# CobaltCrabby/ray_tracer

Hardware: AMD Instinct MI355X
Metric: Mrays/s (reference-semantics closest-hit queries) at 1920x1080 Sponza (higher is better)
Workload: dtype f32; 1 GPU; sponza (synthetic-262267-tris), 1920x1080, 8 spp/step, bounceLimit 8, rows interleaved over 1 GPU(s), up to 10 steps in flight per rank (groups of 10+9+9+9); scene=sponza, assets=synthetic-262267-tris, width=1920, height=1080, frames_in_flight=10, pipeline=multi-kernel (k_trace_pw + k_shade per round)

## Files before the change

ray_tracer_amd/csrc/rt_device.hip:

```cpp

#include "rt_kernels.hip.h"
#include "bvh_build.hip.h"

#include <dlfcn.h>
#include <rccl/rccl.h>

#include <algorithm>
#include <chrono>
#include <cmath>
#include <cstdio>
#include <cstdlib>
#include <string>
#include <type_traits>
#include <vector>

namespace {

struct DevBuf {
    void* p = nullptr;
    size_t bytes = 0;
    DevBuf() = default;
    DevBuf(DevBuf&& o) noexcept : p(o.p), bytes(o.bytes) { o.p = nullptr; o.bytes = 0; }
    ~DevBuf() { release(); }
    void release() { if (p) (void)hipFree(p); p = nullptr; bytes = 0; }
};

struct EventPair { hipEvent_t a, b; };
#define RT_MAX_LANES 4
#define RT_FRAMES_MAX_SLOTS (24ull << 20)
struct RowsOf {
    uint32_t width = 0, height = 0, row0 = 0, rowStride = 0, nRows = 0;
    bool whole(uint32_t w, uint32_t h) const { return width == w && height == h && row0 == 0 && rowStride == 1 && nRows == h; }
};

}

struct rt_ctx {
    std::string error;
    int device = 0, numCUs = 256;
    hipStream_t ownStream = nullptr, stream = nullptr;
    DevScene sc{};
    std::vector<DevBuf> sceneBufs;
    DevBuf texelBuf, texInfoBuf, triUVBuf, objTreeBuf, objCostBuf;
    DevBuf matBuf, sphereBuf, sphereMatBuf, objInvBuf, objFwdBuf, objMetaBuf, objBoxBuf, objSkipBuf, maskBoxBuf, emitBuf, emitPreBuf;
    SceneSources host;
    DevBuf objAlphaBuf;
    uint32_t maxLeafDepth = 0;
    std::vector<RootInfo> rootOf;
    bool cull = false;
    ncclComm_t comm = nullptr;
    int commRanks = 0, commRank = 0;
    DevBuf gatherBuf;
    DevBuf stateBuf, queueBuf, fbBuf, counterBuf, scratchBuf;
    DevBuf overflowBuf[RT_MAX_LANES];
    hipStream_t sideStream[RT_MAX_LANES - 1] = {};
    hipEvent_t forkEvent = nullptr, joinEvent[RT_MAX_LANES - 1] = {}, pollEventSide[RT_MAX_LANES - 1] = {};
    uint32_t capacity = 0;
    PathState ps{}; Queues q{};
    uint32_t* hostCounts = nullptr;
    uint32_t fbPixels = 0; bool fbValid = false;
    bool profiling = false;
    std::vector<EventPair> evPool;
    size_t evUsed = 0;
    hipEvent_t profBase = nullptr;
    DevCounters* snap = nullptr;
    hipEvent_t snapEvent = nullptr;
    hipEvent_t pollEvent = nullptr;
    DevBuf probeBuf;
    DevBuf waveTimeBuf;
    DevBuf aovBuf, aovCounterBuf;
    DevBuf shadeStatBuf;
    uint32_t aovPixels = 0; bool aovValid = false;
    RowsOf fbRows, aovRows;
    DevBuf dnWorkBuf, dnHostBuf, dnOutBuf;
    size_t dnOutPixels = 0; bool dnValid = false;

    struct Tuning {
        int objTreeMin = 48;
        int framesPerLaunch = 0;
        uint64_t framesMaxSlots = RT_FRAMES_MAX_SLOTS;
        int cameraReuse = 1;
        int lightQueries = 1;
        int lanes = 3;
        bool lanesSet = false;
        uint32_t lanesMinSlots = 1u << 20;
        int laneGridPct = 0;
        int traceVariant = 1;
        int pipeline = -1;
        uint32_t fusedBelowPixels = 4000000;
        uint32_t fusedBelowBoxTests = 70;
        int refill = 8;
        int refillMk = 16;
        bool refillMkSet = false;
        int chunk = 256;
        int ldsStackCap = 24;
        int fastLanes = 32;
        bool fastLanesSet = false;
        int wSetup = 16, wLeaf = 16;
        bool wSetupSet = false, wLeafSet = false;
        int wSetupFused = 16, wLeafFused = 24;
        int blocksPerCU = 0;
        int phaseStats = 0;
        int tileSlots = 1;
        int fastShare = 10;
        int maskIdentity = 0;
        int scatter = -1;
        int hotPairs = 2;
        int pixelRefill = 0;
        int batchPixels = 0;
        int batchFixed = 80;
        int fusedMaps = 0;
        int probe = 1;
    } tune;

    struct Measured {
        bool snapPending = false;
        unsigned long long snapBox = 0, snapRays = 0, snapSeg = 0, snapPaths = 0;
        double boxPerRay = -1.0;
        double segPerPath = -1.0;
    } meas;

    struct Reports {
        int lastPipeline = 0;
        int lastParts = 1;
        char lastKernel[96] = "";
        size_t waveTimesCount = 0;
        double traceMs = 0.0;
        uint64_t traceLaunches = 0;
        std::vector<std::pair<float, float>> traceSpans;
        uint64_t traceLaunchesTotal = 0, aovLaunches = 0;
        double bvhBuildMs = 0.0;
    } rep;
    int fail(const std::string& m) { error = m; return -1; }
    int hip(hipError_t e, const char* what) {
        if (e == hipSuccess) return 0;
        error = std::string(what) + ": " + hipGetErrorString(e);
        return -(int)e - 1000;
    }
};

#define RT_HIP(ctx, call)                                    \
    do {                                                     \
        int _rc = (ctx)->hip((call), #call);                 \
        if (_rc) return _rc;                                 \
    } while (0)

namespace {

int dev_alloc(rt_ctx* c, DevBuf& b, size_t bytes) {
    if (b.p && b.bytes >= bytes) return 0;
    b.release();
    if (bytes == 0) bytes = 256;
    RT_HIP(c, hipMalloc(&b.p, bytes));
    b.bytes = bytes;
    return 0;
}

int upload(rt_ctx* c, DevBuf& b, const void* src, size_t bytes) {
    int rc = dev_alloc(c, b, bytes);
    if (rc) return rc;
    if (bytes) RT_HIP(c, hipMemcpyAsync(b.p, src, bytes, hipMemcpyHostToDevice, c->stream));
    RT_HIP(c, hipStreamSynchronize(c->stream));
    return 0;
}

template <typename T>
int upload_table(rt_ctx* c, DevBuf& b, const std::vector<T>& v, const T*& field) {
    int rc = upload(c, b, v.data(), v.size() * sizeof(T));
    if (rc) return rc;
    field = (const T*)b.p;
    return 0;
}

int ensure_state(rt_ctx* c, uint32_t nPixels) {
    if (c->capacity >= nPixels && c->stateBuf.p) return 0;
    const size_t stride4 = (((size_t)nPixels * 16) + 255) & ~(size_t)255;
    const size_t stride1 = (((size_t)nPixels * 4) + 255) & ~(size_t)255;
    const int nF4 = RT_STATE_F4_ARRAYS, nU1 = 2;
    int rc = dev_alloc(c, c->stateBuf, stride4 * nF4 + stride1 * nU1);
    if (rc) return rc;
    PathState& ps = c->ps;
    ps.base = (float4*)c->stateBuf.p;
    ps.pitch = (uint32_t)(stride4 / 16);
    ps.pitchStat = (uint32_t)(stride1 / 4);

    const size_t qa = (((size_t)nPixels * 4) + 255) & ~(size_t)255;
    const size_t qr = (((size_t)nPixels * 3 * 4) + 255) & ~(size_t)255;
    rc = dev_alloc(c, c->queueBuf, 2 * qa + 2 * qr + 256);
    if (rc) return rc;
    char* qb = (char*)c->queueBuf.p;
    c->q.active[0] = (uint32_t*)qb;
    c->q.active[1] = (uint32_t*)(qb + qa);
    c->q.rays[0] = (uint32_t*)(qb + 2 * qa);
    c->q.rays[1] = (uint32_t*)(qb + 2 * qa + qr);
    c->q.counts = (uint32_t*)(qb + 2 * qa + 2 * qr);
// ... 73 lines not shown
    return trace_pw_kernel<STACK, OVF, false, false, CULL>();
}

template <typename K>
uint32_t resident_blocks(const rt_ctx* c, K kernel) {
    int perCU = c->tune.blocksPerCU;
    if (perCU <= 0 && (hipOccupancyMaxActiveBlocksPerMultiprocessor(&perCU, kernel, RT_BLOCK, 0) != hipSuccess || perCU <= 0)) perCU = 4;
    return (uint32_t)perCU * (uint32_t)c->numCUs;
}

int overflow_buf(rt_ctx* c, const Dispatch& d, int stack, bool ovf, uint32_t resident, uint32_t** out) {
    *out = nullptr;
    if (!ovf || c->maxLeafDepth <= (uint32_t)stack) return 0;
    DevBuf& ob = c->overflowBuf[d.part];
    int rc = dev_alloc(c, ob, (size_t)(c->maxLeafDepth - stack) * resident * RT_BLOCK * 4);
    if (rc) return rc;
    *out = (uint32_t*)ob.p;
    return 0;
}

int wave_time_buf(rt_ctx* c, uint32_t blocks, unsigned long long** out) {
    c->rep.waveTimesCount = (size_t)blocks * (RT_BLOCK / RT_WAVE);
    int rc = dev_alloc(c, c->waveTimeBuf, c->rep.waveTimesCount * 16);
    if (rc) return rc;
    *out = (unsigned long long*)c->waveTimeBuf.p;
    return 0;
}

int prof_begin(rt_ctx* c, const Dispatch& d, EventPair** ev) {
    *ev = nullptr;
    if (!d.profiled) return 0;
    if (c->evUsed == c->evPool.size()) {
        EventPair p;
        RT_HIP(c, hipEventCreate(&p.a));
        RT_HIP(c, hipEventCreate(&p.b));
        c->evPool.push_back(p);
    }
    *ev = &c->evPool[c->evUsed++];
    RT_HIP(c, hipEventRecord((*ev)->a, d.stream));
    return 0;
}
int prof_end(rt_ctx* c, const Dispatch& d, EventPair* ev) {
    if (ev) RT_HIP(c, hipEventRecord(ev->b, d.stream));
    if (d.launches) ++*d.launches;
    return 0;
}

uint32_t fused_batch_pixels(const rt_ctx* c, uint32_t nPixels, uint32_t waves, uint32_t evenBelow) {
    if (c->tune.batchPixels > 0) return (uint32_t)std::min(c->tune.batchPixels, (int)RT_WAVE);
    if (((uint64_t)nPixels + RT_WAVE - 1) / RT_WAVE > (uint64_t)evenBelow * waves) return RT_WAVE;
    uint32_t best = RT_WAVE;
    uint64_t bestCost = ~0ull;
    for (uint32_t b = RT_WAVE; b >= 16; b--) {
        const uint64_t nb = (nPixels + b - 1) / b;
        const uint64_t rounds = (nb + waves - 1) / waves;
        const uint64_t cost = rounds * (uint64_t)((uint32_t)c->tune.batchFixed + b);
        if (cost < bestCost) { bestCost = cost; best = b; }
    }
    return best;
}

int launch_fused(rt_ctx* c, const Dispatch& d, const FrameParams& fp, float4* fb) {
    EventPair* ev;
    int rc = prof_begin(c, d, &ev);
    if (rc) return rc;
    const FusedChoice k = d.sc.mapFlags
        ? kernel_choice(d.pixStats ? k_render_fused_maps<true> : k_render_fused_maps<false>, k_render_fused_maps<false>, 24, true, "k_render_fused_maps<%s>", tf(d.pixStats))
        : with_stack<false>(c->maxLeafDepth, (uint32_t)c->tune.ldsStackCap, c->cull, [&](auto S, auto O, auto C) { return d.pixStats ? fused_kernel<S, O, true, C>() : fused_kernel<S, O, false, C>(); });
    const uint32_t resident = resident_blocks(c, k.occupancy);
    const uint32_t nSlots = (uint32_t)dispatch_slots(fp.nPixels, fp.nFrames);
    const uint64_t fewBelow = (c->meas.segPerPath >= 0.0 && c->meas.segPerPath < 2.5) ? 8ull : 5ull;
    const bool fewBlocks = ((uint64_t)nSlots + RT_WAVE - 1) / RT_WAVE < fewBelow * resident * (RT_BLOCK / RT_WAVE);
    const uint32_t pixelRefill = c->tune.pixelRefill > 0 ? (uint32_t)c->tune.pixelRefill
                               : ((c->meas.boxPerRay >= (double)c->tune.fusedBelowBoxTests || fewBlocks) ? 8u : (uint32_t)RT_WAVE);
    const uint32_t evenBelow = pixelRefill < RT_WAVE ? 1u : 2u;
    uint32_t batchPixels = fused_batch_pixels(c, nSlots, resident * (RT_BLOCK / RT_WAVE), evenBelow);
    const uint32_t wavesResident = resident * (RT_BLOCK / RT_WAVE);
    const uint32_t g = fp.nFrames > 1u ? 0u : c->tune.scatter >= 0 ? (uint32_t)c->tune.scatter : ((((uint64_t)nSlots + RT_WAVE - 1) / RT_WAVE <= (uint64_t)evenBelow * wavesResident) ? 4u : 0u);
    if (g) batchPixels = std::min((uint32_t)RT_WAVE, (batchPixels + g - 1) / g * g);
    const uint32_t nBatches = g ? ((nSlots + g - 1) / g + batchPixels / g - 1) / (batchPixels / g) : (nSlots + batchPixels - 1) / batchPixels;
    const uint32_t blocks = std::max(1u, std::min((nBatches + (RT_BLOCK / RT_WAVE) - 1) / (RT_BLOCK / RT_WAVE), resident));
    uint32_t* overflow;
    if ((rc = overflow_buf(c, d, k.stack, k.ovf, resident, &overflow))) return rc;
    RT_HIP(c, hipMemsetAsync(d.counts + 5, 0, 4, d.stream));
    const uint32_t fastLanes = c->tune.fastLanesSet ? (uint32_t)c->tune.fastLanes : (c->meas.boxPerRay >= (double)c->tune.fusedBelowBoxTests ? 40u : 24u);
    const uint32_t wLeaf = (uint32_t)c->tune.wLeafFused;
    unsigned long long* waveTimes = nullptr;
    if (d.phaseStats && (rc = wave_time_buf(c, blocks, &waveTimes))) return rc;
    FusedArgs fa{d.counts + 5, fb, (DevCounters*)c->counterBuf.p, overflow, (uint32_t)c->tune.refill, (uint32_t)c->tune.wSetupFused, wLeaf, fastLanes, batchPixels, g, (uint32_t)c->tune.fastShare, waveTimes, pixelRefill};
    const FusedKernArgs ka{d.sc, c->ps, fp, fa};
    memcpy(c->rep.lastKernel, k.name, sizeof k.name);
    hipLaunchKernelGGL(k.kernel, dim3(blocks), dim3(RT_BLOCK), 0, d.stream, ka);
    RT_HIP(c, hipGetLastError());
    return prof_end(c, d, ev);
}

template <int STACK>
void launch_v0_t(rt_ctx* c, const Dispatch& d, uint32_t maxRays, const TraceArgs& ta) {
    uint32_t blocks = (maxRays + RT_BLOCK - 1) / RT_BLOCK;
    snprintf(c->rep.lastKernel, sizeof c->rep.lastKernel, "k_trace<%d>", STACK);
    hipLaunchKernelGGL((k_trace<STACK>), dim3(blocks), dim3(RT_BLOCK), 0, d.stream, d.sc, c->ps, ta);
}

int launch_trace(rt_ctx* c, const Dispatch& d, uint32_t maxRays, const TraceArgs& ta) {
    if (maxRays == 0) return 0;
    EventPair* ev;
    int rc = prof_begin(c, d, &ev);
    if (rc) return rc;
    const uint32_t depth = c->maxLeafDepth;
    const bool pix = d.pixStats || ta.perRayBox;
    const bool alpha = d.sc.mapFlags & RT_MAP_ALPHA;
    if (!alpha && c->tune.traceVariant == 0) {
        if (depth <= 8) launch_v0_t<8>(c, d, maxRays, ta);
        else if (depth <= 16) launch_v0_t<16>(c, d, maxRays, ta);
        else if (depth <= 24) launch_v0_t<24>(c, d, maxRays, ta);
        else if (depth <= 32) launch_v0_t<32>(c, d, maxRays, ta);
        else if (depth <= 48) launch_v0_t<48>(c, d, maxRays, ta);
        else launch_v0_t<64>(c, d, maxRays, ta);
    } else {
        const bool tableWanted = c->tune.hotPairs && d.sc.hotNodes > 0 && !d.phaseStats && !pix;
        const uint32_t cap = (depth > 24u && c->tune.ldsStackCap >= 24 && tableWanted) ? 16u : (uint32_t)c->tune.ldsStackCap;
        const TracePwChoice k = alpha
            ? kernel_choice(pix ? k_trace_pw_alpha<true> : k_trace_pw_alpha<false>, k_trace_pw_alpha<false>, 24, true, "k_trace_pw_alpha<%s>", tf(pix))
            : with_stack<true>(depth, cap, c->cull, [&](auto S, auto O, auto C) { return choose_trace_pw<S, O, C>(c, d, pix); });
        const uint32_t resident = resident_blocks(c, k.occupancy);
        const uint32_t blocks = std::min((maxRays + RT_BLOCK - 1) / RT_BLOCK, std::max(1u, (uint32_t)((uint64_t)resident * (uint32_t)d.gridPct / 100u)));
        uint32_t* overflow;
        if ((rc = overflow_buf(c, d, k.stack, k.ovf, resident, &overflow))) return rc;
        unsigned long long* waveTimes = nullptr;
        const bool times = d.phaseStats == 1 || (d.phaseStats >= 2 && d.launches && *d.launches == (uint64_t)(d.phaseStats - 2));
        if (!alpha && times && (rc = wave_time_buf(c, blocks, &waveTimes))) return rc;
        const bool longRays = c->meas.boxPerRay >= (double)c->tune.fusedBelowBoxTests;
        const uint32_t refillMk = c->tune.refillMkSet ? (uint32_t)c->tune.refillMk : (longRays ? 12u : 16u);
        const uint32_t wSetup = c->tune.wSetupSet ? (uint32_t)c->tune.wSetup : (longRays ? 32u : 16u);
        const TracePwArgs pa{ta.queue, ta.count, d.counts + 4, refillMk, (uint32_t)c->tune.chunk, wSetup, (uint32_t)c->tune.wLeaf, (uint32_t)c->tune.fastLanes, (uint32_t)c->tune.fastShare,
                             ta.perRayBox, ta.perRayTri, ta.counters, (unsigned long long*)((char*)c->counterBuf.p + sizeof(DevCounters)), waveTimes, overflow, ta.countAux, ta.countAux2, ta.auxOffset};
        memcpy(c->rep.lastKernel, k.name, sizeof k.name);
        hipLaunchKernelGGL(k.kernel, dim3(blocks), dim3(RT_BLOCK), 0, d.stream, d.sc, c->ps, pa);
    }
    RT_HIP(c, hipGetLastError());
    return prof_end(c, d, ev);
}

void poll_ray_cost(rt_ctx* c) {
    if (!c->meas.snapPending || hipEventQuery(c->snapEvent) != hipSuccess) return;
    c->meas.snapPending = false;
    const unsigned long long box = c->snap->boxTests - c->snap->skippedBoxTests, rays = c->snap->raysTraced;
    if (rays > c->meas.snapRays && box >= c->meas.snapBox && rays - c->meas.snapRays > 100000ull)
        c->meas.boxPerRay = (double)(box - c->meas.snapBox) / (double)(rays - c->meas.snapRays);
    const unsigned long long seg = c->snap->segments, paths = c->snap->paths;
    if (paths > c->meas.snapPaths && seg >= c->meas.snapSeg && paths - c->meas.snapPaths > 100000ull) c->meas.segPerPath = (double)(seg - c->meas.snapSeg) / (double)(paths - c->meas.snapPaths);
    c->meas.snapBox = box;
    c->meas.snapRays = rays;
    c->meas.snapSeg = seg;
    c->meas.snapPaths = paths;
}
void request_ray_cost(rt_ctx* c) {
    if (c->meas.snapPending) return;
    if (hipMemcpyAsync(c->snap, c->counterBuf.p, sizeof(DevCounters), hipMemcpyDeviceToHost, c->stream) != hipSuccess) return;
    if (hipEventRecord(c->snapEvent, c->stream) != hipSuccess) return;
    c->meas.snapPending = true;
}
void measured_new_scene(rt_ctx* c) {
    if (c->meas.snapPending) { c->meas.snapBox = c->snap->boxTests; c->meas.snapRays = c->snap->raysTraced; c->meas.snapPending = false; }
    c->meas.boxPerRay = -1.0;
}

int harvest_events(rt_ctx* c) {
    for (size_t i = 0; i < c->evUsed; i++) {
        float ms = 0.f;
        RT_HIP(c, hipEventElapsedTime(&ms, c->evPool[i].a, c->evPool[i].b));
        c->rep.traceMs += ms;
        c->rep.traceLaunches++;
        float t0 = 0.f;
        if (c->profBase && hipEventElapsedTime(&t0, c->profBase, c->evPool[i].a) == hipSuccess) c->rep.traceSpans.emplace_back(t0, t0 + ms);
    }
    c->evUsed = 0;
    return 0;
}

int rebuild_emitters(rt_ctx* c) {
    c->sc.emitCount = 0; c->sc.emitSphereMask = 0; c->sc.emitMode = 0;
    const MapLayout maps = layout_maps(c->host, c->sc.texCount);
    int rc = upload_table(c, c->objAlphaBuf, maps.objAlpha, c->sc.objAlpha);
    if (rc) return rc;
    c->sc.mapFlags = maps.mapFlags;
    if (!c->tune.lightQueries) return 0;
    const EmitterLayout e = layout_emitters(c->host, c->rootOf, c->sc.texCount);
    if (!e.mode) return 0;
    if (!e.tris.empty()) {
        if ((rc = upload_table(c, c->emitBuf, e.tris, c->sc.emitTris))) return rc;
    } else {
        if ((rc = dev_alloc(c, c->emitBuf, 256))) return rc;
        c->sc.emitTris = (const uint2*)c->emitBuf.p;
    }
    if ((rc = dev_alloc(c, c->emitPreBuf, std::max<size_t>(e.tris.size(), 1) * 4 * sizeof(float4)))) return rc;
    if (!e.tris.empty()) {
        hipLaunchKernelGGL(k_emit_precompute, dim3(((uint32_t)e.tris.size() + 63u) / 64u), dim3(64), 0, c->stream, c->sc.triPos, c->sc.emitTris, (uint32_t)e.tris.size(), (float4*)c->emitPreBuf.p);
        RT_HIP(c, hipGetLastError());
        RT_HIP(c, hipStreamSynchronize(c->stream));
    }
    c->sc.emitPre = (const float4*)c->emitPreBuf.p;
    c->sc.emitCount = (uint32_t)e.tris.size();
    c->sc.emitSphereMask = e.sphereMask;
    c->sc.emitMode = 1;
    return 0;
}

int set_materials(rt_ctx* c, const RayMaterial* m, uint32_t n) {
    int rc = upload_table(c, c->matBuf, layout_materials(m, n), c->sc.mats);
    if (rc) return rc;
    c->sc.materialCount = n;
    c->host.mats.assign(m, m + n);
    return rebuild_emitters(c);
}

int set_spheres(rt_ctx* c, const Sphere* s, uint32_t n) {
    const SphereLayout l = layout_spheres(s, n);
    int rc = upload_table(c, c->sphereBuf, l.spheres, c->sc.spheres);
    if (rc) return rc;
    if ((rc = upload_table(c, c->sphereMatBuf, l.mat, c->sc.sphereMat))) return rc;
    c->sc.sphereCount = n;
    c->sc.sphereTestMask = l.testMask;
    c->host.sphereMat.assign(l.mat.begin(), l.mat.begin() + n);
    return rebuild_emitters(c);
}

int set_objects(rt_ctx* c, const ObjectLayout& l, const RenderObject* o, uint32_t n) {
    if (l.treeLevels && getenv("RT_DEBUG_OBJTREE")) dump_object_tree(l, n);
    int rc;
    if ((rc = upload_table(c, c->objInvBuf, l.inv, c->sc.objInv))) return rc;
    if ((rc = upload_table(c, c->objFwdBuf, l.fwd, c->sc.objFwd))) return rc;
    if ((rc = upload_table(c, c->objMetaBuf, l.meta, c->sc.objMeta))) return rc;
    if ((rc = upload_table(c, c->objBoxBuf, l.box, c->sc.objBox))) return rc;
    if ((rc = upload_table(c, c->maskBoxBuf, l.maskBox, c->sc.maskBox))) return rc;
    if ((rc = upload_table(c, c->objSkipBuf, l.skipCost, c->sc.objSkipCost))) return rc;
    if ((rc = upload_table(c, c->objTreeBuf, l.tree, c->sc.objTree))) return rc;
    if ((rc = upload_table(c, c->objCostBuf, l.cost, c->sc.objCost))) return rc;
    for (int k = 0; k <= RT_OBJTREE_LEVELS; k++) c->sc.objTreeOff[k] = l.treeOff[k];
    c->sc.objTreeLevels = l.treeLevels;
    c->sc.reachCount = l.reachCount;
    c->sc.maskBase = l.maskBase;
    c->sc.cullOriginLimit = l.cullOriginLimit;
    c->cull = l.cull;
    c->sc.objectCount = n;
    c->host.objMat.resize(n); c->host.objRoot.resize(n); c->host.objSampler.resize(n);
    for (uint32_t i = 0; i < n; i++) { c->host.objMat[i] = o[i].materialIndex; c->host.objRoot[i] = o[i].bvhIndex; c->host.objSampler[i] = o[i].samplerIndex; }
    return rebuild_emitters(c);
}

}

extern "C" {

int rt_device_count(int* out) {
    int n = 0;
    hipError_t e = hipGetDeviceCount(&n);
    if (out) *out = (e == hipSuccess) ? n : 0;
    return e == hipSuccess ? 0 : -1;
}

int rt_create(int device, rt_ctx** out) {
    if (!out) return -1;
    *out = nullptr;
    int n = 0;
    if (hipGetDeviceCount(&n) != hipSuccess || n <= 0) return -2;
    if (device < 0 || device >= n) return -3;
    if (hipSetDevice(device) != hipSuccess) return -4;
    rt_ctx* c = new rt_ctx();
    c->device = device;
    if (hipStreamCreateWithFlags(&c->ownStream, hipStreamNonBlocking) != hipSuccess) { c->ownStream = nullptr; rt_destroy(c); return -5; }
    c->stream = c->ownStream;
    {
        hipDeviceProp_t prop;
        if (hipGetDeviceProperties(&prop, device) == hipSuccess && prop.multiProcessorCount > 0) c->numCUs = prop.multiProcessorCount;
    }
    if (hipHostMalloc((void**)&c->hostCounts, 64, hipHostMallocDefault) != hipSuccess) { c->hostCounts = nullptr; rt_destroy(c); return -6; }
    if (hipHostMalloc((void**)&c->snap, sizeof(DevCounters), hipHostMallocDefault) != hipSuccess) { c->snap = nullptr; rt_destroy(c); return -6; }
    if (hipEventCreateWithFlags(&c->snapEvent, hipEventDisableTiming) != hipSuccess) { c->snapEvent = nullptr; rt_destroy(c); return -6; }
    if (hipEventCreateWithFlags(&c->pollEvent, hipEventDisableTiming) != hipSuccess) { c->pollEvent = nullptr; rt_destroy(c); return -6; }
    if (dev_alloc(c, c->counterBuf, sizeof(DevCounters) + 256) != 0) { rt_destroy(c); return -7; }
    (void)hipMemsetAsync(c->counterBuf.p, 0, sizeof(DevCounters) + 256, c->stream);
    if (dev_alloc(c, c->aovCounterBuf, sizeof(DevCounters)) != 0) { rt_destroy(c); return -7; }
    (void)hipMemsetAsync(c->aovCounterBuf.p, 0, sizeof(DevCounters), c->stream);
    if (dev_alloc(c, c->shadeStatBuf, sizeof(ShadeStatStripe) * RT_STAT_STRIPES) != 0) { rt_destroy(c); return -7; }
    (void)hipMemsetAsync(c->shadeStatBuf.p, 0, sizeof(ShadeStatStripe) * RT_STAT_STRIPES, c->stream);
    (void)hipStreamSynchronize(c->stream);
    *out = c;
    return 0;
}

void rt_destroy(rt_ctx* c) {
    if (!c) return;
    (void)hipSetDevice(c->device);
    if (c->stream) (void)hipStreamSynchronize(c->stream);
    (void)rt_comm_destroy(c);
    for (auto& e : c->evPool) { (void)hipEventDestroy(e.a); (void)hipEventDestroy(e.b); }
    if (c->hostCounts) (void)hipHostFree(c->hostCounts);
    if (c->snap) (void)hipHostFree(c->snap);
    for (hipEvent_t e : {c->snapEvent, c->pollEvent, c->forkEvent, c->profBase})
        if (e) (void)hipEventDestroy(e);
    for (int l = 0; l < RT_MAX_LANES - 1; l++) {
        if (c->joinEvent[l]) (void)hipEventDestroy(c->joinEvent[l]);
        if (c->pollEventSide[l]) (void)hipEventDestroy(c->pollEventSide[l]);
        if (c->sideStream[l]) (void)hipStreamDestroy(c->sideStream[l]);
    }
    if (c->ownStream) (void)hipStreamDestroy(c->ownStream);
    delete c;
}

const char* rt_last_error(const rt_ctx* c) { return c ? c->error.c_str() : "null ctx"; }

int rt_set_stream(rt_ctx* c, void* s) {
    if (!c) return -1;
    RT_HIP(c, hipStreamSynchronize(c->stream));
    c->stream = s ? (hipStream_t)s : c->ownStream;
    return 0;
}

int rt_upload_textures(rt_ctx* c, const RtTexture* tex, uint32_t n) {
    if (!c || (!tex && n)) return -1;
    const TextureLayout l = layout_textures(tex, n);
    if (!l.error.empty()) return c->fail(l.error);
    RT_HIP(c, hipSetDevice(c->device));
    int rc = upload_table(c, c->texelBuf, l.texels, c->sc.texels);
    if (rc) return rc;
    if ((rc = upload_table(c, c->texInfoBuf, l.info, c->sc.texInfo))) return rc;
    c->sc.texCount = n;
    return rebuild_emitters(c);
}

int rt_update_materials(rt_ctx* c, const RayMaterial* m, uint32_t n) {
    if (!c || (!m && n)) return -1;
    RT_HIP(c, hipSetDevice(c->device));
    return set_materials(c, m, n);
}

int rt_update_spheres(rt_ctx* c, const Sphere* s, uint32_t n) {
    if (!c || (!s && n)) return -1;
    RT_HIP(c, hipSetDevice(c->device));
    return set_spheres(c, s, n);
}

int rt_update_objects(rt_ctx* c, const RenderObject* o, uint32_t n) {
    if (!c || (!o && n)) return -1;
    if (c->rootOf.empty() && n) return c->fail("rt_update_objects before rt_upload_scene");
    const ObjectLayout l = layout_objects(o, n, c->rootOf, c->sc.materialCount, c->tune.objTreeMin, c->tune.maskIdentity);
    if (!l.error.empty()) return c->fail(l.error);
    RT_HIP(c, hipSetDevice(c->device));
    return set_objects(c, l, o, n);
}

int rt_upload_scene(rt_ctx* c, const RtSceneArrays* s) {
    if (!c || !s) return -1;
    SceneLayout l = layout_scene(*s, c->tune.objTreeMin, c->tune.maskIdentity);
    if (!l.error.empty()) return c->fail(l.error);
    MeshLayout& m = l.meshes;

    RT_HIP(c, hipSetDevice(c->device));
    RT_HIP(c, hipStreamSynchronize(c->stream));
    measured_new_scene(c);
    c->host = SceneSources{};
    c->sc.emitMode = 0; c->sc.emitCount = 0; c->sc.emitSphereMask = 0;
    c->sc.mapFlags = 0;
    c->sc.texCount = 0;
    c->sceneBufs.clear();
    c->sceneBufs.resize(5);
    int rc;
    if ((rc = upload_table(c, c->triUVBuf, m.triUV, c->sc.triUV))) return rc;
// ... 8 lines not shown
    c->maxLeafDepth = m.maxLeafDepth;
    c->rootOf = std::move(m.rootOf);

    if ((rc = set_materials(c, s->materials, s->materialCount))) return rc;
    if ((rc = set_spheres(c, s->spheres, s->sphereCount))) return rc;
    return set_objects(c, l.objects, s->objects, s->objectCount);
}

int rt_sync(rt_ctx* c) {
    if (!c) return -1;
    RT_HIP(c, hipStreamSynchronize(c->stream));
    return harvest_events(c);
}

}

namespace {
int check_tile(rt_ctx* c, const PushConstants* pc, uint32_t width, uint32_t height, uint32_t row0, uint32_t rowStride, uint32_t nRows,
               const char* fn) {
    if (width == 0 || height == 0 || rowStride == 0) return c->fail(std::string(fn) + ": bad image geometry");
    if (nRows && (uint64_t)row0 + (uint64_t)(nRows - 1) * rowStride >= height) return c->fail(std::string(fn) + ": rows exceed the image");
    if (!c->sc.nodes) return c->fail(std::string(fn) + " before rt_upload_scene");
    const RayTracerData& td = pc->rayTraceParams;
    if (td.sphereCount > c->sc.sphereCount) return c->fail("rayTraceParams.sphereCount exceeds the uploaded spheres");
    if (td.objectCount > c->sc.objectCount) return c->fail("rayTraceParams.objectCount exceeds the uploaded objects");
    return 0;
}

DevScene dispatch_scene(const rt_ctx* c, const RayTracerData& td) {
    DevScene sc = c->sc;
    sc.sphereCount = td.sphereCount;
    sc.objectCount = td.objectCount;
    if (sc.objectCount < c->sc.objectCount) { sc.reachCount = 0; sc.objTreeLevels = 0; }
    return sc;
}

FrameParams frame_camera(const rt_ctx* c, const PushConstants* pc, uint32_t width, uint32_t height, uint32_t row0, uint32_t rowStride,
                         uint32_t nRows, uint32_t nPixels) {
    FrameParams fp{};
    memcpy(fp.camRot, pc->camInfo.cameraRotation, 64);
    memcpy(fp.camPos, pc->camInfo.pos, 12);
    fp.planeHeight = pc->camInfo.nearPlane * rt_tan(rt_radians(pc->camInfo.fov * 0.5f)) * 2.f;
    fp.planeWidth = fp.planeHeight * pc->camInfo.aspectRatio;
    fp.bottomLeft[0] = -fp.planeWidth / 2.f;
    fp.bottomLeft[1] = -fp.planeHeight / 2.f;
    fp.bottomLeft[2] = 0.1f;
    fp.tiled = (c->tune.tileSlots && (width % 8u) == 0u) ? 1u : 0u;
    fp.width = width; fp.height = height; fp.row0 = row0; fp.rowStride = rowStride; fp.nRows = nRows; fp.nPixels = nPixels;
    return fp;
}

int choose_pipeline(const rt_ctx::Tuning& t, int pipeline, double boxPerRay, const DevScene& sc, uint32_t nSlots) {
    const bool shortRays = boxPerRay >= 0.0 && boxPerRay < (double)t.fusedBelowBoxTests;
    double sizeLimit = (double)t.fusedBelowPixels;
    if (boxPerRay > 90.0) sizeLimit = std::max(0.375 * sizeLimit, sizeLimit - (boxPerRay - 90.0) * (0.625 / 60.0) * sizeLimit);
    const bool bigScene = (uint64_t)sc.nodeCount * 32u + (uint64_t)sc.triCount * 48u > (4ull << 20);
    const bool shortButMissing = shortRays && bigScene && boxPerRay >= 25.0 && nSlots >= (10u << 20);
    const int chosen = pipeline >= 0 ? pipeline : (((double)nSlots < sizeLimit || (shortRays && !shortButMissing)) ? 1 : 0);
    return (sc.mapFlags && !t.fusedMaps) ? 0 : chosen;
}

int choose_parts(const rt_ctx::Tuning& t, const Dispatch& d, bool cull, double boxPerRay, uint32_t samples, uint32_t nSlots) {
    int nLanes = (samples > 0 && nSlots >= t.lanesMinSlots) ? std::max(1, std::min(t.lanes, (int)RT_MAX_LANES)) : 1;
    if (d.phaseStats) nLanes = 1;
    if (!t.lanesSet && cull && boxPerRay >= 150.0 && nSlots >= (8u << 20)) nLanes = 1;
    return nLanes;
}
int part_grid_pct(const rt_ctx::Tuning& t, int nLanes, uint32_t firstPartSlots) {
    return nLanes > 1 ? (t.laneGridPct > 0 ? t.laneGridPct : (firstPartSlots < 1200000u ? 40 : 50)) : 100;
}

int ensure_part_streams(rt_ctx* c, int nLanes) {
    for (int l = 1; l < nLanes; l++) {
        if (!c->sideStream[l - 1]) {
            if (hipStreamCreateWithFlags(&c->sideStream[l - 1], hipStreamNonBlocking) != hipSuccess) { c->sideStream[l - 1] = nullptr; nLanes = l; break; }
            if (hipEventCreateWithFlags(&c->joinEvent[l - 1], hipEventDisableTiming) != hipSuccess ||
                hipEventCreateWithFlags(&c->pollEventSide[l - 1], hipEventDisableTiming) != hipSuccess) { nLanes = l; break; }
        }
    }
    if (nLanes > 1 && !c->forkEvent && hipEventCreateWithFlags(&c->forkEvent, hipEventDisableTiming) != hipSuccess) { c->forkEvent = nullptr; nLanes = 1; }
    return nLanes;
}

struct Lane { Dispatch d; hipEvent_t poll; uint32_t begin, n, ubActive; int cur; bool pollPending, done; };
void slice_parts(rt_ctx* c, const Dispatch& d, uint32_t nSlots, uint32_t nFrames, int nLanes, Lane* lane) {
    const uint32_t unit = 256u * std::max(1u, nFrames);
    const uint32_t units = (nSlots + unit - 1) / unit;
    uint32_t at = 0;
    for (int l = 0; l < nLanes; l++) {
        const uint32_t u = units / (uint32_t)nLanes + ((uint32_t)l < units % (uint32_t)nLanes ? 1u : 0u);
        const uint32_t end = std::min(nSlots, at + u * unit);
        lane[l] = Lane{d, l ? c->pollEventSide[l - 1] : c->pollEvent, at, end - at, end - at, 0, false, end == at};
        lane[l].d.stream = l ? c->sideStream[l - 1] : c->stream; lane[l].d.counts = c->q.counts + 16 * l; lane[l].d.part = l;
        at = end;
    }
    const int gridPct = part_grid_pct(c->tune, nLanes, lane[0].n);
    for (int l = 0; l < nLanes; l++) lane[l].d.gridPct = gridPct;
}

int render_rounds(rt_ctx* c, const FrameParams& fp, Lane* lane, int nLanes) {
    DevCounters* dc = (DevCounters*)c->counterBuf.p;
    int rc = 0;
    if (nLanes > 1) {
        RT_HIP(c, hipEventRecord(c->forkEvent, c->stream));
        for (int l = 1; l < nLanes; l++) RT_HIP(c, hipStreamWaitEvent(lane[l].d.stream, c->forkEvent, 0));
    }
    const uint64_t maxRounds = (uint64_t)fp.samples * ((uint64_t)fp.bounceLimit + 1);
    for (uint64_t it = 0; it < maxRounds; it++) {
        bool any = false;
        for (int l = 0; l < nLanes; l++) {
            Lane& L = lane[l];
            if (L.done) continue;
            any = true;
            const hipStream_t stream = L.d.stream; uint32_t* const counts = L.d.counts;
            const int cur = L.cur, nxt = cur ^ 1;
            uint32_t* const active[2] = {c->q.active[0] + L.begin, c->q.active[1] + L.begin};
            uint32_t* const rays[2] = {c->q.rays[0] + 3 * (size_t)L.begin, c->q.rays[1] + 3 * (size_t)L.begin};
            hipLaunchKernelGGL(k_zero_counts, dim3(1), dim3(64), 0, stream, counts + nxt, counts + 2 + nxt, counts + 4, counts + 5 + nxt, counts + 7 + nxt);
            TraceArgs ta{rays[cur], counts + 2 + cur, nullptr, nullptr, dc, counts + 5 + cur, counts + 7 + cur, L.n};
            const uint64_t ubRays = std::min<uint64_t>((uint64_t)L.ubActive * 3, (uint64_t)L.n * 3);
            if ((rc = launch_trace(c, L.d, (uint32_t)ubRays, ta))) break;
            ShadeArgs sa{active[cur], counts + cur, active[nxt], rays[nxt], counts + nxt, counts + 2 + nxt, (ShadeStatStripe*)c->shadeStatBuf.p, counts + 5 + nxt, counts + 7 + nxt, L.n};
            if (L.d.sc.mapFlags & (RT_MAP_METALNESS | RT_MAP_BUMP)) hipLaunchKernelGGL(k_shade_maps, dim3((L.ubActive + RT_BLOCK - 1) / RT_BLOCK), dim3(RT_BLOCK), 0, stream, L.d.sc, c->ps, sa, fp);
            else hipLaunchKernelGGL(k_shade, dim3((L.ubActive + RT_BLOCK - 1) / RT_BLOCK), dim3(RT_BLOCK), 0, stream, L.d.sc, c->ps, sa, fp);
            L.cur = nxt;
            if (L.pollPending && hipEventQuery(L.poll) == hipSuccess) {
                L.pollPending = false;
                L.ubActive = std::min(L.ubActive, c->hostCounts[8 + l]);
                if (L.ubActive == 0) { L.done = true; continue; }
            }
            if (!L.pollPending && (it & 7u) == 7u) {
                if (hipMemcpyAsync(c->hostCounts + 8 + l, counts + L.cur, 4, hipMemcpyDeviceToHost, stream) == hipSuccess &&
                    hipEventRecord(L.poll, stream) == hipSuccess)
                    L.pollPending = true;
            }
        }
        if (!any || rc) break;
    }
    for (int l = 1; l < nLanes; l++) {
        RT_HIP(c, hipEventRecord(c->joinEvent[l - 1], lane[l].d.stream));
        RT_HIP(c, hipStreamWaitEvent(c->stream, c->joinEvent[l - 1], 0));
    }
    hipLaunchKernelGGL(k_fold_shade_stats, dim3(1), dim3(RT_STAT_STRIPES), 0, c->stream, (ShadeStatStripe*)c->shadeStatBuf.p, dc);
    return rc;
}

int render_parts(rt_ctx* c, const FrameParams& fp, const Dispatch& d, uint32_t nSlots, float4* fb) {
    const int nLanes = ensure_part_streams(c, choose_parts(c->tune, d, c->cull, c->meas.boxPerRay, fp.samples, nSlots));
    c->rep.lastParts = nLanes;
    Lane lane[RT_MAX_LANES];
    slice_parts(c, d, nSlots, fp.nFrames, nLanes, lane);
    for (int l = 0; l < nLanes; l++) {
        const Lane& L = lane[l];
        if (!L.n) continue;
        hipLaunchKernelGGL(k_raygen, dim3((L.n + RT_BLOCK - 1) / RT_BLOCK), dim3(RT_BLOCK), 0, c->stream, d.sc, c->ps,
                           c->q.active[0] + L.begin, c->q.rays[0] + 3 * (size_t)L.begin, fp, L.begin, L.begin + L.n);
        if (fp.samples > 0) hipLaunchKernelGGL(k_init_counts, dim3(1), dim3(64), 0, c->stream, L.d.counts, L.n);
    }
    RT_HIP(c, hipGetLastError());
    if (fp.samples > 0)
        if (int rc = render_rounds(c, fp, lane, nLanes)) return rc;
    const uint32_t blocksPix = (fp.nPixels + RT_BLOCK - 1) / RT_BLOCK;
    if (fp.nFrames > 1u) hipLaunchKernelGGL(k_blend_frames, dim3(blocksPix), dim3(RT_BLOCK), 0, c->stream, c->ps, fp, fb);
    else hipLaunchKernelGGL(k_resolve, dim3(blocksPix), dim3(RT_BLOCK), 0, c->stream, c->ps, fp, fb);
    RT_HIP(c, hipGetLastError());
    return 0;
}

int probe_ray_cost(rt_ctx* c, const FrameParams& fp, const Dispatch& d);

int render_dispatch(rt_ctx* c, const FrameParams& fp, const Dispatch& d, float4* fb) {
    const uint32_t nSlots = (uint32_t)dispatch_slots(fp.nPixels, fp.nFrames);
    int rc;
    poll_ray_cost(c);
    if (c->meas.boxPerRay < 0.0 && c->tune.probe && !d.probe && !d.sc.mapFlags && (uint64_t)fp.nPixels * fp.samples >= 8000000ull && fp.debug < 0 &&
        (rc = probe_ray_cost(c, fp, d)))
        return rc;
    const int pipeline = choose_pipeline(c->tune, d.pipeline, c->meas.boxPerRay, d.sc, nSlots);
    if (!d.probe) c->rep.lastPipeline = pipeline;
    if (pipeline == 1) {
        rc = launch_fused(c, d, fp, fb);
        if (!rc && fp.nFrames > 1u) {
            hipLaunchKernelGGL(k_blend_frames, dim3((fp.nPixels + RT_BLOCK - 1) / RT_BLOCK), dim3(RT_BLOCK), 0, c->stream, c->ps, fp, fb);
            rc = c->hip(hipGetLastError(), "k_blend_frames");
        }
    } else {
        rc = render_parts(c, fp, d, nSlots, fb);
    }
    if (!rc) request_ray_cost(c);
    return rc;
}

int probe_ray_cost(rt_ctx* c, const FrameParams& fp, const Dispatch& d) {
    const uint32_t rows = std::min(fp.nRows, 8u), skip = fp.nRows / rows;
    FrameParams p = fp;
    p.samples = 1; p.progressive = 0; p.debug = -1; p.nFrames = 1;
    p.row0 = fp.row0 + (skip / 2u) * fp.rowStride; p.rowStride = fp.rowStride * skip; p.nRows = rows; p.nPixels = rows * fp.width;
    Dispatch pd = d;
    pd.probe = true; pd.pipeline = 1; pd.profiled = false; pd.phaseStats = 0; pd.launches = nullptr;
    int rc = dev_alloc(c, c->probeBuf, (size_t)rows * fp.width * sizeof(float4));
    if (rc) return rc;
    DevCounters before, after;
    RT_HIP(c, hipMemcpyAsync(&before, c->counterBuf.p, sizeof(DevCounters), hipMemcpyDeviceToHost, c->stream));
    RT_HIP(c, hipStreamSynchronize(c->stream));
    if ((rc = render_dispatch(c, p, pd, (float4*)c->probeBuf.p))) return rc;
    RT_HIP(c, hipMemcpyAsync(&after, c->counterBuf.p, sizeof(DevCounters), hipMemcpyDeviceToHost, c->stream));
    RT_HIP(c, hipStreamSynchronize(c->stream));
    RT_HIP(c, hipMemcpyAsync(c->counterBuf.p, &before, sizeof(DevCounters), hipMemcpyHostToDevice, c->stream));
    RT_HIP(c, hipStreamSynchronize(c->stream));
    c->meas.snapPending = false;
    if (after.raysTraced > before.raysTraced + 1000ull)
        c->meas.boxPerRay = (double)((after.boxTests - after.skippedBoxTests) - (before.boxTests - before.skippedBoxTests)) / (double)(after.raysTraced - before.raysTraced);
    return 0;
}

int render_impl(rt_ctx* c, const PushConstants* pc, uint32_t width, uint32_t height, uint32_t row0, uint32_t rowStride,
                uint32_t nRows, uint32_t nFrames, float* d_rgba) {
    if (!c || !pc) return -1;
    int rc = check_tile(c, pc, width, height, row0, rowStride, nRows, "rt_render");
    if (rc) return rc;
    const RayTracerData& td = pc->rayTraceParams;
    if (td.bounceLimit >= (1u << 28) - 1u) return c->fail("rayTraceParams.bounceLimit needs more than 28 bits");
    const uint64_t np64 = (uint64_t)nRows * width;
    if (frame_slots(np64) * nFrames >= (1ull << 30)) return c->fail("tile too large (slot ids are 30 bits)");
    const uint32_t nPixels = (uint32_t)np64;
    RT_HIP(c, hipSetDevice(c->device));
// ... 30 lines not shown
}

extern "C" {

int rt_render(rt_ctx* c, const PushConstants* pc, uint32_t width, uint32_t height, uint32_t row0, uint32_t rowStride,
              uint32_t nRows, float* d_rgba) {
    return render_impl(c, pc, width, height, row0, rowStride, nRows, 1u, d_rgba);
}

int rt_render_frames(rt_ctx* c, const PushConstants* pc, uint32_t width, uint32_t height, uint32_t row0, uint32_t rowStride,
                     uint32_t nRows, uint32_t nFrames, float* d_rgba) {
    if (!c || !pc) return -1;
    if (nFrames == 0) return 0;
    const uint64_t np = (uint64_t)nRows * width;
    uint32_t per = 1;
    if (nFrames > 1u && pc->rayTraceParams.debug < 0 && np > 0) {
        const uint64_t cap = std::min<uint64_t>(std::max<uint64_t>(c->tune.framesMaxSlots, np), (1ull << 30) - 1);
        per = (uint32_t)std::max<uint64_t>(1, std::min<uint64_t>(nFrames, cap / frame_slots(np)));
        if (c->tune.framesPerLaunch > 0) per = std::min(per, (uint32_t)c->tune.framesPerLaunch);
    }
    PushConstants p = *pc;
    for (uint32_t f = 0; f < nFrames; f += per) {
        const uint32_t n = std::min(per, nFrames - f);
        p.frameCount = pc->frameCount + f;
        int rc = render_impl(c, &p, width, height, row0, rowStride, nRows, n, d_rgba);
        if (rc) return rc;
    }
    return 0;
}

int rt_clear_framebuffer(rt_ctx* c) {
    if (!c) return -1;
    c->fbPixels = 0;
    c->fbValid = false;
    return 0;
}

int rt_read_rgba_f32(rt_ctx* c, float* out, size_t nFloats) {
    if (!c || !out) return -1;
    if (!c->fbValid) return c->fail("no ctx-owned framebuffer: rt_render was never called with d_rgba = NULL");
    if (nFloats != (size_t)c->fbPixels * 4) return c->fail("rt_read_rgba_f32: size mismatch");
    RT_HIP(c, hipSetDevice(c->device));
    RT_HIP(c, hipMemcpyAsync(out, c->fbBuf.p, nFloats * 4, hipMemcpyDeviceToHost, c->stream));
    RT_HIP(c, hipStreamSynchronize(c->stream));
    return 0;
}

int rt_read_rgba8_srgb(rt_ctx* c, uint8_t* out, size_t nBytes) {
    if (!c || !out) return -1;
    if (!c->fbValid || nBytes != (size_t)c->fbPixels * 4) return c->fail("rt_read_rgba8_srgb: size mismatch");
    std::vector<float> tmp((size_t)c->fbPixels * 4);
    int rc = rt_read_rgba_f32(c, tmp.data(), tmp.size());
    if (rc) return rc;
    for (size_t i = 0; i < tmp.size(); i++) {
        float v = tmp[i];
        if (!(v > 0.f)) v = 0.f;
        if (v > 1.f) v = 1.f;
        if ((i & 3) != 3) v = v <= 0.0031308f ? 12.92f * v : 1.055f * rt_pow(v, 1.f / 2.4f) - 0.055f;
        out[i] = (uint8_t)(v * 255.f + 0.5f);
    }
    return 0;
}

int rt_trace_rays(rt_ctx* c, uint32_t n, const float* origins, const float* dirs, RtHit* hitsOut) {
    if (!c || !origins || !dirs || !hitsOut) return -1;
    if (!c->sc.nodes) return c->fail("rt_trace_rays before rt_upload_scene");
    if (n == 0) return 0;
    RT_HIP(c, hipSetDevice(c->device));
    int rc = ensure_state(c, n);
    if (rc) return rc;
    std::vector<float4> ho(n), hd(n);
    for (uint32_t i = 0; i < n; i++) {
        ho[i] = make_float4(origins[(size_t)i * 3], origins[(size_t)i * 3 + 1], origins[(size_t)i * 3 + 2], 0.f);
        hd[i] = make_float4(dirs[(size_t)i * 3], dirs[(size_t)i * 3 + 1], dirs[(size_t)i * 3 + 2], 0.f);
    }
    RT_HIP(c, hipMemcpyAsync(c->ps.rayO(), ho.data(), (size_t)n * 16, hipMemcpyHostToDevice, c->stream));
    RT_HIP(c, hipMemcpyAsync(c->ps.rayD(), hd.data(), (size_t)n * 16, hipMemcpyHostToDevice, c->stream));
    RT_HIP(c, hipStreamSynchronize(c->stream));
    size_t need = (size_t)n * 8 + (size_t)n * sizeof(RtHit) + 256;
    if ((rc = dev_alloc(c, c->scratchBuf, need))) return rc;
    uint32_t* prb = (uint32_t*)c->scratchBuf.p;
    uint32_t* prt = prb + n;
    RtHit* dh = (RtHit*)((char*)c->scratchBuf.p + (((size_t)n * 8 + 255) & ~(size_t)255));
    c->hostCounts[0] = n; c->hostCounts[1] = 0; c->hostCounts[2] = 0; c->hostCounts[3] = 0; c->hostCounts[4] = 0;
    RT_HIP(c, hipMemcpyAsync(c->q.counts, c->hostCounts, 20, hipMemcpyHostToDevice, c->stream));
    RT_HIP(c, hipMemsetAsync(c->ps.statBox(), 0, (size_t)n * 4, c->stream));
    RT_HIP(c, hipMemsetAsync(c->ps.statTri(), 0, (size_t)n * 4, c->stream));
    hipLaunchKernelGGL(k_seed_rays, dim3((n + RT_BLOCK - 1) / RT_BLOCK), dim3(RT_BLOCK), 0, c->stream, c->sc, c->ps, n);
    TraceArgs ta{nullptr, c->q.counts, prb, prt, (DevCounters*)c->counterBuf.p};
    if ((rc = launch_trace(c, one_part(c, c->sc, false), n, ta))) return rc;
    hipLaunchKernelGGL(k_hit_details, dim3((n + RT_BLOCK - 1) / RT_BLOCK), dim3(RT_BLOCK), 0, c->stream, c->sc, c->ps, n, prb, prt, dh);
    RT_HIP(c, hipGetLastError());
    RT_HIP(c, hipMemcpyAsync(hitsOut, dh, (size_t)n * sizeof(RtHit), hipMemcpyDeviceToHost, c->stream));
    RT_HIP(c, hipStreamSynchronize(c->stream));
    return harvest_events(c);
}

int rt_render_aovs(rt_ctx* c, const PushConstants* pc, uint32_t width, uint32_t height, uint32_t row0, uint32_t rowStride,
                   uint32_t nRows, const RtAovBuffers* d_out) {
    if (!c || !pc) return -1;
    int rc = check_tile(c, pc, width, height, row0, rowStride, nRows, "rt_render_aovs");
    if (rc) return rc;
    const uint64_t np64 = (uint64_t)nRows * width;
    if (np64 >= (1ull << 30)) return c->fail("rt_render_aovs: tile too large (slot ids are 30 bits)");
    const uint32_t nPixels = (uint32_t)np64;
    RT_HIP(c, hipSetDevice(c->device));
    if (nPixels == 0) return 0;
    if (c->capacity < nPixels || !c->stateBuf.p) RT_HIP(c, hipStreamSynchronize(c->stream));
    if ((rc = ensure_state(c, nPixels))) return rc;
    AovOut out;
    if (d_out) {
        out = AovOut{(float4*)d_out->normalDepth, (float4*)d_out->position, (float4*)d_out->albedo, (float4*)d_out->rayDir, (uint4*)d_out->ids};
    } else {
        if ((rc = dev_alloc(c, c->aovBuf, (size_t)nPixels * sizeof(float4) * 5))) return rc;
        float4* p = (float4*)c->aovBuf.p;
        out = AovOut{p, p + nPixels, p + 2 * (size_t)nPixels, p + 3 * (size_t)nPixels, (uint4*)(p + 4 * (size_t)nPixels)};
        c->aovPixels = nPixels;
        c->aovValid = true;
        c->aovRows = RowsOf{width, height, row0, rowStride, nRows};
    }
    FrameParams fp = frame_camera(c, pc, width, height, row0, rowStride, nRows, nPixels);
    fp.nFrames = 1;
    Dispatch d = one_part(c, dispatch_scene(c, pc->rayTraceParams), false);
    d.phaseStats = 0; d.launches = &c->rep.aovLaunches;
    const uint32_t blocks = (nPixels + RT_BLOCK - 1) / RT_BLOCK;
    hipLaunchKernelGGL(k_aov_rays, dim3(blocks), dim3(RT_BLOCK), 0, c->stream, d.sc, c->ps, fp);
    hipLaunchKernelGGL(k_init_counts, dim3(1), dim3(64), 0, c->stream, c->q.counts, nPixels);
    RT_HIP(c, hipGetLastError());
    const TraceArgs ta{nullptr, c->q.counts, nullptr, nullptr, (DevCounters*)c->aovCounterBuf.p};
    if ((rc = launch_trace(c, d, nPixels, ta))) return rc;
    hipLaunchKernelGGL(k_aov_resolve, dim3(blocks), dim3(RT_BLOCK), 0, c->stream, d.sc, c->ps, fp, out);
    RT_HIP(c, hipGetLastError());
    return 0;
}

int rt_read_aovs(rt_ctx* c, const RtAovBuffers* out, size_t nPixels) {
    if (!c || !out) return -1;
    if (!c->aovValid) return c->fail("no ctx-owned AOV planes: rt_render_aovs was never called with d_out = NULL");
    if (nPixels != (size_t)c->aovPixels) return c->fail("rt_read_aovs: size mismatch");
    RT_HIP(c, hipSetDevice(c->device));
    const float4* p = (const float4*)c->aovBuf.p;
    void* const dst[5] = {out->normalDepth, out->position, out->albedo, out->rayDir, out->ids};
    for (int k = 0; k < 5; k++)
        if (dst[k]) RT_HIP(c, hipMemcpyAsync(dst[k], p + (size_t)k * nPixels, nPixels * sizeof(float4), hipMemcpyDeviceToHost, c->stream));
    RT_HIP(c, hipStreamSynchronize(c->stream));
    return 0;
}
}

namespace {
int check_denoise(rt_ctx* c, uint32_t width, uint32_t height, const RtDenoiseParams& p, const char* fn) {
    const std::string f(fn);
    if (width == 0 || height == 0) return c->fail(f + ": bad image geometry");
    if ((uint64_t)width * height >= (1ull << 30) || height > 65535u * 16u) return c->fail(f + ": image too large");
    if (p.iterations > 10) return c->fail(f + ": iterations must be 0..10");
    if (!(std::isfinite(p.sigmaLuminance) && p.sigmaLuminance > 0.f)) return c->fail(f + ": sigmaLuminance must be finite and > 0");
    if (!(std::isfinite(p.sigmaNormal) && p.sigmaNormal >= 0.f)) return c->fail(f + ": sigmaNormal must be finite and >= 0");
    if (!(std::isfinite(p.sigmaDepth) && p.sigmaDepth > 0.f)) return c->fail(f + ": sigmaDepth must be finite and > 0");
    if (!c->sc.nodes) return c->fail(f + " before rt_upload_scene");
    return 0;
}

std::string not_whole(const char* what, const RowsOf& r, uint32_t width, uint32_t height) {
    char m[256];
    snprintf(m, sizeof(m), "rt_denoise: %s: rows %u + k*%u, k < %u of a %u x %u image, not the whole %u x %u frame", what, r.row0,
             r.rowStride, r.nRows, r.width, r.height, width, height);
    return m;
}

bool overlap(const void* a, const void* b, size_t bytes) {
    const uintptr_t x = (uintptr_t)a, y = (uintptr_t)b;
    return x < y + bytes && y < x + bytes;
}
}

extern "C" {

void rt_denoise_params_default(RtDenoiseParams* p) {
    if (p) *p = RtDenoiseParams{5u, 4.f, 128.f, 1.f};
}

int rt_denoise(rt_ctx* c, uint32_t width, uint32_t height, const float* d_rgba, const RtAovBuffers* d_aovs, const RtDenoiseParams* params,
               float* d_out) {
    if (!c) return -1;
    RtDenoiseParams p;
    rt_denoise_params_default(&p);
    if (params) p = *params;
    int rc = check_denoise(c, width, height, p, "rt_denoise");
    if (rc) return rc;
    const size_t n = (size_t)width * height, bytes = n * sizeof(float4);
    const float4* rgba = (const float4*)d_rgba;
    if (!rgba) {
        if (!c->fbValid) return c->fail("rt_denoise: no ctx-owned framebuffer: rt_render was never called with d_rgba = NULL");
        if (!c->fbRows.whole(width, height)) return c->fail(not_whole("the ctx framebuffer", c->fbRows, width, height));
        rgba = (const float4*)c->fbBuf.p;
    }
    const float4 *nd, *albedo;
    const uint4* ids;
    if (!d_aovs) {
        if (!c->aovValid) return c->fail("rt_denoise: no ctx-owned AOV planes: rt_render_aovs was never called with d_out = NULL");
        if (!c->aovRows.whole(width, height)) return c->fail(not_whole("the ctx AOV planes", c->aovRows, width, height));
        const float4* a = (const float4*)c->aovBuf.p;
        nd = a;
        albedo = a + 2 * n;
        ids = (const uint4*)(a + 4 * n);
    } else {
        if (!d_aovs->normalDepth || !d_aovs->albedo || !d_aovs->ids) return c->fail("rt_denoise: d_aovs needs the normalDepth, albedo and ids planes");
        nd = (const float4*)d_aovs->normalDepth;
        albedo = (const float4*)d_aovs->albedo;
        ids = (const uint4*)d_aovs->ids;
    }
    if (d_out)
        for (const void* in : {(const void*)rgba, (const void*)nd, (const void*)albedo, (const void*)ids})
// ... 93 lines not shown
                ps[0] ? (double)ps[16] / ps[0] : 0.0, ps[1] ? (double)ps[17] / ps[1] : 0.0, ps[2] ? (double)ps[18] / ps[2] : 0.0, ps[3] ? (double)ps[19] / ps[3] : 0.0);
        fprintf(stderr, "[phase_stats] trips of the set-up step's object-skipping loop: %llu (%.1f per lane and set-up step)\n", ps[20], ps[5] ? (double)ps[20] / ps[5] : 0.0);
        fprintf(stderr, "[phase_stats] lanes sitting out interior rounds: %.1f at a leaf, %.1f in set-up states, %.1f without a ray (of 64, average)\n",
                ps[2] ? (double)ps[12] / ps[2] : 0.0, ps[2] ? (double)ps[13] / ps[2] : 0.0, ps[2] ? (double)ps[14] / ps[2] : 0.0);
        if (c->rep.waveTimesCount && c->waveTimeBuf.p) {
            std::vector<unsigned long long> t(c->rep.waveTimesCount * 2);
            RT_HIP(c, hipMemcpy(t.data(), c->waveTimeBuf.p, t.size() * 8, hipMemcpyDeviceToHost));
            unsigned long long t0 = ~0ull, t1 = 0;
            for (size_t w = 0; w < c->rep.waveTimesCount; w++) { t0 = std::min(t0, t[2 * w]); t1 = std::max(t1, t[2 * w + 1]); }
            std::vector<double> end(c->rep.waveTimesCount);
            double busy = 0;
            const double span = (double)(t1 - t0);
            for (size_t w = 0; w < c->rep.waveTimesCount; w++) { end[w] = (t[2 * w + 1] - t0) / span; busy += (t[2 * w + 1] - t[2 * w]) / span; }
            std::sort(end.begin(), end.end());
            auto q = [&](double f) { return end[std::min(end.size() - 1, (size_t)(f * end.size()))]; };
            fprintf(stderr, "[phase_stats] last launch: %zu waves, span %.3f ms (100 MHz clock), mean wave lifetime %.1f %% of it; waves finished by 10/25/50/75/90/99 %% : %.2f %.2f %.2f %.2f %.2f %.2f of the span\n",
                    c->rep.waveTimesCount, span / 1e5, 100.0 * busy / c->rep.waveTimesCount, q(0.10), q(0.25), q(0.50), q(0.75), q(0.90), q(0.99));
        }
    }
    return 0;
}

int rt_reset_counters(rt_ctx* c) {
    if (!c) return -1;
    RT_HIP(c, hipSetDevice(c->device));
    RT_HIP(c, hipStreamSynchronize(c->stream));
    poll_ray_cost(c);
    RT_HIP(c, hipMemsetAsync(c->counterBuf.p, 0, sizeof(DevCounters) + 256, c->stream));
    RT_HIP(c, hipMemsetAsync(c->aovCounterBuf.p, 0, sizeof(DevCounters), c->stream));
    RT_HIP(c, hipStreamSynchronize(c->stream));
    c->meas.snapPending = false;
    c->meas.snapBox = 0; c->meas.snapRays = 0; c->meas.snapSeg = 0; c->meas.snapPaths = 0;
    int rc = harvest_events(c);
    c->rep.traceMs = 0.0; c->rep.traceLaunches = 0; c->rep.traceLaunchesTotal = 0; c->rep.aovLaunches = 0;
    c->rep.traceSpans.clear();
    return rc;
}

int rt_set_profiling(rt_ctx* c, int on) {
    if (!c) return -1;
    RT_HIP(c, hipStreamSynchronize(c->stream));
    int rc = harvest_events(c);
    c->profiling = on != 0;
    if (on) {
        if (!c->profBase) RT_HIP(c, hipEventCreate(&c->profBase));
        RT_HIP(c, hipEventRecord(c->profBase, c->stream));
        c->rep.traceSpans.clear();
    }
    return rc;
}

int rt_get_trace_busy_ms(rt_ctx* c, double* ms) {
    if (!c || !ms) return -1;
    RT_HIP(c, hipStreamSynchronize(c->stream));
    int rc = harvest_events(c);
    std::vector<std::pair<float, float>> v = c->rep.traceSpans;
    std::sort(v.begin(), v.end());
    double busy = 0.0, end = -1e300;
    for (const auto& iv : v) {
        if ((double)iv.first > end) { busy += (double)iv.second - (double)iv.first; end = iv.second; }
        else if ((double)iv.second > end) { busy += (double)iv.second - end; end = iv.second; }
    }
    *ms = busy;
    return rc;
}

int rt_get_trace_time_ms(rt_ctx* c, double* ms, uint64_t* launches) {
    if (!c) return -1;
    RT_HIP(c, hipStreamSynchronize(c->stream));
    int rc = harvest_events(c);
    if (ms) *ms = c->rep.traceMs;
    if (launches) *launches = c->rep.traceLaunches;
    return rc;
}

const char* rt_last_kernel(const rt_ctx* c) { return c ? c->rep.lastKernel : ""; }
int rt_last_parts(const rt_ctx* c) { return c ? c->rep.lastParts : 0; }

int rt_set_tuning(rt_ctx* c, const char* key, int value) {
    if (!c || !key) return -1;
    std::string k(key);
    if (k == "pipeline") { if (value < -1 || value > 1) return c->fail("pipeline: -1 (auto), 0 or 1"); c->tune.pipeline = value; }
    else if (k == "probe") { c->tune.probe = value ? 1 : 0; }
    else if (k == "frames_max_mslots") { if (value < 1 || value > 1000) return c->fail("frames_max_mslots: 1..1000 (millions of paths per multi-frame dispatch)"); c->tune.framesMaxSlots = (uint64_t)value << 20; }
    else if (k == "frames_per_launch") { if (value < 0) return c->fail("frames_per_launch >= 0"); c->tune.framesPerLaunch = value; }
    else if (k == "camera_reuse") { c->tune.cameraReuse = value ? 1 : 0; }
    else if (k == "light_queries") { c->tune.lightQueries = value ? 1 : 0; int rc = rebuild_emitters(c); if (rc) return rc; }
    else if (k == "fused_below_box_tests") { if (value < 0) return c->fail("fused_below_box_tests >= 0"); c->tune.fusedBelowBoxTests = (uint32_t)value; }
    else if (k == "fused_below_pixels") { if (value < 0) return c->fail("fused_below_pixels >= 0"); c->tune.fusedBelowPixels = (uint32_t)value; }
    else if (k == "trace_variant") { if (value < 0 || value > 1) return c->fail("trace_variant: 0 or 1"); c->tune.traceVariant = value; }
    else if (k == "refill") { if (value < 1 || value > 64) return c->fail("refill: 1..64"); c->tune.refill = value; c->tune.refillMk = value; c->tune.refillMkSet = true; }
    else if (k == "hot_pairs") { if (value < 0 || value > 2) return c->fail("hot_pairs: 0, 1 (six work-groups per CU) or 2 (five)"); c->tune.hotPairs = value; }
    else if (k == "mk_refill") { if (value < 1 || value > 64) return c->fail("mk_refill: 1..64"); c->tune.refillMk = value; c->tune.refillMkSet = true; }
    else if (k == "lds_stack") { if (value != 8 && value != 16 && value != 24) return c->fail("lds_stack: 8, 16 or 24"); c->tune.ldsStackCap = value; }
    else if (k == "fast_lanes") { if (value < 0 || value > 65) return c->fail("fast_lanes: 1..65 (0: back to the defaults)"); c->tune.fastLanesSet = value != 0; c->tune.fastLanes = value ? value : 32; }
    else if (k == "chunk") { if (value < 1 || value > 4096) return c->fail("chunk: 1..4096"); c->tune.chunk = value; }
    else if (k == "w_setup") { if (value < 1 || value > 512) return c->fail("w_setup: 1..512"); c->tune.wSetup = value; c->tune.wSetupFused = value; c->tune.wSetupSet = true; }
    else if (k == "w_leaf") { if (value < 1 || value > 512) return c->fail("w_leaf: 1..512"); c->tune.wLeaf = value; c->tune.wLeafFused = value; c->tune.wLeafSet = true; }
    else if (k == "mk_w_setup") { if (value < 1 || value > 512) return c->fail("mk_w_setup: 1..512"); c->tune.wSetup = value; c->tune.wSetupSet = true; }
    else if (k == "mk_w_leaf") { if (value < 1 || value > 512) return c->fail("mk_w_leaf: 1..512"); c->tune.wLeaf = value; }
    else if (k == "tile_slots") { c->tune.tileSlots = value != 0; }
    else if (k == "mask_identity") { c->tune.maskIdentity = value != 0; }
    else if (k == "fast_share") { if (value < 0 || value > 16) return c->fail("fast_share: 0..16"); c->tune.fastShare = value; }
    else if (k == "scatter") { if (value != -1 && value != 0 && value != 1 && value != 2 && value != 4 && value != 8 && value != 16) return c->fail("scatter: -1 (auto), 0, 1, 2, 4, 8 or 16"); c->tune.scatter = value; }
    else if (k == "fused_maps") { if (value < 0 || value > 1) return c->fail("fused_maps: 0 (map scenes take the multi-kernel pipeline) or 1 (they choose as usual)"); c->tune.fusedMaps = value; }
    else if (k == "pixel_refill") { if (value < 0 || value > (int)RT_WAVE) return c->fail("pixel_refill must be 0 (by ray length) .. 64"); c->tune.pixelRefill = value; }
    else if (k == "batch_pixels") { if (value < 0 || value > (int)RT_WAVE) return c->fail("batch_pixels must be 0 (auto) .. 64"); c->tune.batchPixels = value; }
    else if (k == "batch_fixed") { if (value < 0 || value > 4096) return c->fail("batch_fixed out of range"); c->tune.batchFixed = value; }
    else if (k == "phase_stats") { if (value < 0) return c->fail("phase_stats >= 0"); c->tune.phaseStats = value; }
    else if (k == "object_tree_min") { if (value < 0) return c->fail("object_tree_min >= 0"); c->tune.objTreeMin = value; }
    else if (k == "lanes") { if (value < 0 || value > RT_MAX_LANES) return c->fail("lanes: 1..4 (parts of a multi-kernel dispatch, each on its own stream), 0 = automatic"); c->tune.lanes = value ? value : 3; c->tune.lanesSet = value != 0; }
    else if (k == "lane_grid_pct") { if (value != 0 && (value < 10 || value > 100)) return c->fail("lane_grid_pct: 0 (by size) or 10..100"); c->tune.laneGridPct = value; }
    else if (k == "lanes_min_kslots") { if (value < 0) return c->fail("lanes_min_kslots >= 0"); c->tune.lanesMinSlots = (uint32_t)value << 10; }
    else if (k == "blocks_per_cu") { if (value < 0 || value > 8) return c->fail("blocks_per_cu: 0..8"); c->tune.blocksPerCU = value; }
    else return c->fail("unknown tuning key " + k);
    return 0;
}

int rt_last_pipeline(const rt_ctx* c) { return c ? c->rep.lastPipeline : -1; }
double rt_ray_cost(const rt_ctx* c) { return c ? c->meas.boxPerRay : -1.0; }

int rt_bvh_build(rt_ctx* c, const TrianglePoint* points, uint32_t pointCount, Triangle* triangles, float* centroids, uint32_t count,
                 uint32_t triIndex0, uint32_t nodeBase, BVHNode* nodesOut, uint32_t nodeCapacity, uint32_t* nodeCountOut, uint32_t statsOut[3]) {
    if (!c || !points || !triangles || !centroids || !nodesOut || !nodeCountOut) return -1;
    if (count == 0) return c->fail("rt_bvh_build: a mesh with 0 triangles");
    if (nodeCapacity < 2u * count - 1u) return c->fail("rt_bvh_build: node capacity below 2 * count - 1");
    RT_HIP(c, hipSetDevice(c->device));
    const auto t0 = std::chrono::steady_clock::now();
    const bool dbg = getenv("RT_BVH_DEBUG") != nullptr;
    auto mark = [&](const char* what) { if (dbg) fprintf(stderr, "[rt_bvh_build] %-12s %8.2f ms\n", what, std::chrono::duration<double, std::milli>(std::chrono::steady_clock::now() - t0).count()); };
    std::vector<float> verts((size_t)count * 9);
    for (uint32_t i = 0; i < count; i++) {
        const uint32_t vi[3] = {triangles[i].v0, triangles[i].v1, triangles[i].v2};
        for (int k = 0; k < 3; k++) {
            if (vi[k] >= pointCount) return c->fail("rt_bvh_build: triangle point index out of range");
            memcpy(&verts[(size_t)i * 9 + 3 * k], points[vi[k]].position, 12);
        }
    }
    const size_t nNodesMax = 2 * (size_t)count - 1;
    DevBuf bVerts, bCent, bPerm, bTmp, bHole, bNodes, bList, bCtr, bWide;
    const uint32_t maxChunks = (count + RT_BVH_CHUNK - 1) / RT_BVH_CHUNK;
    int rc;
    if ((rc = upload(c, bVerts, verts.data(), verts.size() * 4)) || (rc = upload(c, bCent, centroids, (size_t)count * 12)) ||
        (rc = dev_alloc(c, bPerm, (size_t)count * 4)) || (rc = dev_alloc(c, bTmp, (size_t)count * 4)) || (rc = dev_alloc(c, bHole, (size_t)count * 4)) ||
        (rc = dev_alloc(c, bNodes, nNodesMax * sizeof(BNode))) || (rc = dev_alloc(c, bList, 2 * (size_t)(count + 1) * 4)) || (rc = dev_alloc(c, bCtr, 64)) ||
        (rc = dev_alloc(c, bWide, RT_BVH_WIDE_NODES * sizeof(WideAcc) + (size_t)RT_BVH_WIDE_NODES * maxChunks * 4)))
        return rc;
    mark("uploaded");
    BvhBuildArgs a{(const float*)bVerts.p, (const float*)bCent.p, (uint32_t*)bPerm.p, (uint32_t*)bTmp.p, (uint32_t*)bHole.p, (BNode*)bNodes.p, (uint32_t*)bCtr.p};
    uint32_t* lists[2] = {(uint32_t*)bList.p, (uint32_t*)bList.p + (count + 1)};
    uint32_t* nextCount = (uint32_t*)bCtr.p + 1;
    hipLaunchKernelGGL(k_bvh_root, dim3(1), dim3(RT_BVH_BLOCK), 0, c->stream, a, count);
    uint32_t zero = 0, nCur = 1;
    hipError_t e = hipMemcpyAsync(lists[0], &zero, 4, hipMemcpyHostToDevice, c->stream);
    int cur = 0;
    std::vector<uint32_t> levelStart{0u, 1u};
    for (uint32_t level = 0; e == hipSuccess && nCur && level <= 64; level++) {
        e = hipMemsetAsync(nextCount, 0, 4, c->stream);
        if (e != hipSuccess) break;
        if (nCur <= RT_BVH_WIDE_NODES && count >= 8192u) {
            const WideArgs w{a, lists[cur], (WideAcc*)bWide.p, (uint32_t*)((char*)bWide.p + RT_BVH_WIDE_NODES * sizeof(WideAcc)), maxChunks, lists[cur ^ 1], nextCount};
            const dim3 gc(maxChunks, nCur), gn(nCur);
            hipLaunchKernelGGL(w_init, gn, dim3(64), 0, c->stream, w);
            hipLaunchKernelGGL(w_minmax, gc, dim3(256), 0, c->stream, w);
            hipLaunchKernelGGL(w_bins, gc, dim3(256), 0, c->stream, w);
            hipLaunchKernelGGL(w_sweep, gn, dim3(64), 0, c->stream, w);
// ... 289 lines not shown
```

ray_tracer_amd/csrc/rt_fused_body.hip.inc:

```

    const DevScene& sc = ka.sc;
    const PathState& ps = ka.ps;
    const FrameParams& fp = ka.fp;
    const FusedArgs& fa = ka.fa;
    __shared__ uint32_t s_stack[(RT_BLOCK / RT_WAVE) * (STACK + 1) * RT_WAVE];
    __shared__ uint32_t s_list[RT_BLOCK / RT_WAVE][3 * RT_WAVE];
    __shared__ float4 s_box[64];
    __shared__ uint2 s_meta[RT_META_LDS];
    const uint32_t nBox = CULL ? sc.reachCount : 0u;
    if (CULL && threadIdx.x < 2u * nBox) s_box[threadIdx.x] = sc.maskBox[threadIdx.x];
    fill_meta_lds(sc, s_meta);
    const uint32_t wv = threadIdx.x / RT_WAVE;
    uint32_t* stack = s_stack + wv * (STACK + 1) * RT_WAVE + (threadIdx.x & (RT_WAVE - 1));
    uint32_t* list = s_list[wv];
    uint32_t* ovf = OVF ? fa.overflow + (size_t)blockIdx.x * RT_BLOCK + threadIdx.x : nullptr;
    const size_t ovfStride = (size_t)gridDim.x * RT_BLOCK;
    const TracePwArgs ta{nullptr, nullptr, nullptr, fa.refill, 0u, fa.wSetup, fa.wLeaf, fa.fastLanes, fa.fastShare, nullptr, nullptr, fa.counters, nullptr, nullptr, fa.overflow};
    WaveTotals wt;
    uint32_t refTot = 0, pathTot = 0, segTot = 0, emitTot = 0;
    const unsigned long long tKernelStart = fa.waveTimes ? wall_clock64() : 0ull;
    const uint32_t nBatches = fa.scatter ? ((fp.nPixels + fa.scatter - 1) / fa.scatter + fa.batchPixels / fa.scatter - 1) / (fa.batchPixels / fa.scatter)
                                         : ((fp.nFrames > 1u ? ((fp.nPixels + 63u) >> 6) * 64u * fp.nFrames : fp.nPixels) + fa.batchPixels - 1) / fa.batchPixels;

    const uint32_t nSlots = fp.nFrames > 1u ? ((fp.nPixels + 63u) >> 6) * 64u * fp.nFrames : fp.nPixels;
    const uint32_t total = fa.scatter ? nBatches * fa.batchPixels : nSlots;
    const uint32_t refillAt = min(max(fa.pixelRefill, 1u), fa.batchPixels);
    uint32_t slot = 0;
    bool valid = false, alive = false, exhausted = false;
    uint32_t auxMask = 0;
    for (;;) {
        const bool mine = lane_id() < fa.batchPixels && !alive;
        const unsigned long long mF = __ballot(mine);
        const uint32_t take = __popcll(mF);
        if (!exhausted && take >= refillAt) {
            uint32_t base = 0;
            if (lane_id() == 0) base = atomicAdd(fa.batchHead, take);
            base = __shfl(base, 0, RT_WAVE);
            if (base >= total) exhausted = true;
            else if (mine) {
                const FusedKernArgs* kq = opaque_kernarg<FusedKernArgs>();
                const FrameParams* fq = &kq->fp;
                const DevScene* sq = &kq->sc;
                if (valid && fq->nFrames == 1u) resolve_pixel(ps, *fq, fa.rgba, slot);
                const uint32_t a = base + lanes_below(mF);
                uint32_t ns = a;
                if (fa.scatter) {
                    const uint32_t ch = a / fa.scatter, perBlock = fa.batchPixels / fa.scatter;
                    ns = ((ch % perBlock) * nBatches + ch / perBlock) * fa.scatter + a % fa.scatter;
                }
                valid = a < total && ns < nSlots && (fq->nFrames == 1u || slot_in_tile(*fq, ns) < fq->nPixels);
                slot = ns;
                auxMask = 0;
                if (valid) {
                    init_path(*sq, ps, *fq, slot);
                    alive = fp.samples > 0;
                }
            }
        }
        const unsigned long long mA = __ballot(alive);
        if (mA == 0) {
            if (exhausted) break;
            continue;
        }
        const unsigned long long mM = __ballot(alive && !(auxMask & 4u));
        const unsigned long long mL = __ballot(alive && (auxMask & 1u)), mC = __ballot(alive && (auxMask & 2u));
        const uint32_t nM = __popcll(mM), nL = __popcll(mL), nC = __popcll(mC);
        if (alive) {
            if (!(auxMask & 4u)) list[lanes_below(mM)] = (slot << 2) | RAY_MAIN;
            if (auxMask & 1u) list[nM + lanes_below(mL)] = (slot << 2) | RAY_NEE;
            if (auxMask & 2u) list[nM + nL + lanes_below(mC)] = (slot << 2) | RAY_PROBE;
        }
        const uint32_t nRays = nM + nL + nC;
        __threadfence_block();
        trace_wave<STACK, OVF, PIX, false, true, CULL, 0, false, ALPHA>(sc, ps, ta, stack, ovf, ovfStride, list, nRays, wt, s_meta);
        __threadfence_block();
        if (alive) {
            bool nowAlive = false;
            uint32_t refRays = 0, nPaths = 0;
            const FusedKernArgs* kq = opaque_kernarg<FusedKernArgs>();
            const FrameParams* fq = &kq->fp;
            const DevScene* sq = &kq->sc;
            shade_path<MAPS>(*sq, ps, *fq, slot, nowAlive, auxMask, refRays, nPaths, emitTot, false);
            segTot++;
            if (CULL && nowAlive && nBox) {
                float4 sd;
                if (!(auxMask & 4u)) {
                    sd = ps.hit(RAY_MAIN)[slot];
                    sd.z = __uint_as_float(reach_mask_from(s_box, nBox, f4xyz(ps.rayO()[slot]), f4xyz(ps.rayD()[slot]), sc.cullOriginLimit));
                    ps.hit(RAY_MAIN)[slot] = sd;
                }
                if (auxMask & 1u) {
                    sd = ps.hit(RAY_NEE)[slot];
                    sd.z = __uint_as_float(reach_mask_from(s_box, nBox, f4xyz(ps.auxO()[slot]), f4xyz(ps.auxDL()[slot]), sc.cullOriginLimit));
                    ps.hit(RAY_NEE)[slot] = sd;
                }
                if (auxMask & 2u) {
                    sd = ps.hit(RAY_PROBE)[slot];
                    sd.z = __uint_as_float(reach_mask_from(s_box, nBox, f4xyz(ps.auxO()[slot]), f4xyz(ps.auxDC()[slot]), sc.cullOriginLimit));
                    ps.hit(RAY_PROBE)[slot] = sd;
                }
// ... 33 lines not shown
```

ray_tracer_amd/csrc/rt_kernels.hip.h:

```cpp
#pragma once

#include <hip/hip_runtime.h>
#include <stdint.h>

#include "rt_amd.h"
#include "rt_det_math.h"
#include "rt_probe.h"
#include "scene_layout.h"

#define RT_WAVE 64
#ifndef RT_QUEUE_ORDER
#define RT_QUEUE_ORDER 0
#endif
#ifndef RT_TE_REG
#define RT_TE_REG 1
#endif
#ifndef RT_OBJTREE
#define RT_OBJTREE 1
#endif
#ifndef RT_SHADE_IDENT
#define RT_SHADE_IDENT 1
#endif
#ifndef RT_FUSED_MAPS_BLOCKS
#define RT_FUSED_MAPS_BLOCKS 4
// ... 18 lines not shown
    uint32_t sphereCount, objectCount, materialCount, nodeCount, triCount;
    uint32_t hotNodes;
    uint32_t sphereTestMask;
    const float4* maskBox;
    const uint2* objSkipCost;
    uint32_t reachCount;
    const float4* objTree;
    const uint2* objCost;
    uint32_t objTreeOff[RT_OBJTREE_LEVELS + 1];
    uint32_t objTreeLevels;
    uint32_t maskBase;
    const uint2* emitTris;
    const float4* emitPre;
    uint32_t emitCount, emitSphereMask, emitMode;
    const uint32_t* texels;
    const uint4* texInfo;
    const float4* triUV;
    uint32_t texCount;
    const uint32_t* objAlpha;
    uint32_t mapFlags;
    float cullOriginLimit;
};

enum { RAY_MAIN = 0, RAY_NEE = 1, RAY_PROBE = 2 };
#define RAY_MAIN_BLANK 3u
__host__ __device__ __forceinline__ uint32_t ray_kind(uint32_t id) { return (id & 3u) == RAY_MAIN_BLANK ? (uint32_t)RAY_MAIN : (id & 3u); }

#define RT_STATE_F4_ARRAYS 15
struct PathState {
    float4* base;
    uint32_t pitch;
    uint32_t pitchStat;
    __host__ __device__ __forceinline__ float4* arr(uint32_t k) const { return base + (size_t)k * pitch; }
    __host__ __device__ __forceinline__ float4* rayO() const { return arr(0); }
    __host__ __device__ __forceinline__ float4* rayD() const { return arr(1); }
    __host__ __device__ __forceinline__ float4* auxO() const { return arr(2); }
    __host__ __device__ __forceinline__ float4* auxDL() const { return arr(3); }
    __host__ __device__ __forceinline__ float4* auxDC() const { return arr(4); }
    __host__ __device__ __forceinline__ float4* hit(uint32_t kind) const { return arr(5 + kind); }
    __host__ __device__ __forceinline__ float4* att() const { return arr(8); }
    __host__ __device__ __forceinline__ float4* total() const { return arr(9); }
    __host__ __device__ __forceinline__ float4* pendAlbedo() const { return arr(10); }
    __host__ __device__ __forceinline__ float4* accum() const { return arr(11); }
    __host__ __device__ __forceinline__ float4* camHit() const { return arr(12); }
    __host__ __device__ __forceinline__ float4* camDir() const { return arr(13); }
    __host__ __device__ __forceinline__ float4* pendMis() const { return arr(14); }
    __host__ __device__ __forceinline__ uint32_t* statBox() const { return (uint32_t*)arr(RT_STATE_F4_ARRAYS); }
    __host__ __device__ __forceinline__ uint32_t* statTri() const { return (uint32_t*)arr(RT_STATE_F4_ARRAYS) + pitchStat; }
};

struct Queues {
    uint32_t* active[2];
    uint32_t* rays[2];
    uint32_t* counts;
};

struct FrameParams {
    float camRot[16];
    float camPos[3];
    float planeWidth, planeHeight;
    float bottomLeft[3];
    uint32_t width, height, row0, rowStride, nRows, nPixels;
    uint32_t tiled;
    uint32_t startingSeed;
    uint32_t samples, bounceLimit;
    uint32_t progressive, frameCount;
    uint32_t camReuse;
    uint32_t nFrames;
    int32_t debug;
    uint32_t boxCap, triCap;
    EnvironmentData env;
};

struct DevCounters {
    unsigned long long boxTests, triTests, raysTraced, raysHit, raysReference, paths, segments, emitterTests;
    unsigned long long skippedBoxTests;
};

#define RT_STAT_STRIPES 256u
struct ShadeStatStripe {
    unsigned long long raysReference, paths, segments, emitterTests;
    unsigned long long pad[12];
};

#define RT_AS_CONSTANT __attribute__((address_space(4)))
#define RT_AS_GLOBAL __attribute__((address_space(1)))
#define RT_AS_LDS __attribute__((address_space(3)))
typedef float rt_f4v __attribute__((ext_vector_type(4)));
typedef float rt_f2v __attribute__((ext_vector_type(2)));
template <typename T> __device__ __forceinline__ const T* rt_uniform(const T* p) { return (const T*)(const RT_AS_CONSTANT T*)(unsigned long long)p; }
template <typename T> __device__ __forceinline__ const T* rt_global(const T* p) { return (const T*)(const RT_AS_GLOBAL T*)(unsigned long long)p; }

__device__ __forceinline__ rt_vec3 f4xyz(float4 v) { return rt_v3(v.x, v.y, v.z); }
__device__ __forceinline__ float4 mk4(rt_vec3 v, float w) { return make_float4(v.x, v.y, v.z, w); }
__device__ __forceinline__ float4 mk4u(rt_vec3 v, uint32_t w) { return make_float4(v.x, v.y, v.z, __uint_as_float(w)); }

__device__ __forceinline__ rt_vec3 xform_dir_rows(float4 r0, float4 r1, float4 r2, rt_vec3 v) {
    return rt_v3((r0.x * v.x + r0.y * v.y) + r0.z * v.z, (r1.x * v.x + r1.y * v.y) + r1.z * v.z,
                 (r2.x * v.x + r2.y * v.y) + r2.z * v.z);
}
__device__ __forceinline__ rt_vec3 xform_point_rows(float4 r0, float4 r1, float4 r2, rt_vec3 v) {
    return rt_v3(((r0.x * v.x + r0.y * v.y) + r0.z * v.z) + r0.w, ((r1.x * v.x + r1.y * v.y) + r1.z * v.z) + r1.w,
                 ((r2.x * v.x + r2.y * v.y) + r2.z * v.z) + r2.w);
}

__device__ __forceinline__ uint32_t lane_id() { return __lane_id(); }
__device__ __forceinline__ uint32_t lanes_below(unsigned long long m) {
    return __builtin_amdgcn_mbcnt_hi((uint32_t)(m >> 32), __builtin_amdgcn_mbcnt_lo((uint32_t)m, 0u));
}
__device__ __forceinline__ unsigned long long wave_sum_u64(unsigned long long v) {
#pragma unroll
    for (int o = 32; o > 0; o >>= 1) v += __shfl_xor(v, o, RT_WAVE);
    return v;
}
__device__ __forceinline__ uint32_t wave_sum_u32(uint32_t v) {
#pragma unroll
    for (int o = 32; o > 0; o >>= 1) v += __shfl_xor(v, o, RT_WAVE);
    return v;
}

struct SphereHit { bool didHit, frontFace; float dst; };

__device__ __forceinline__ SphereHit sphere_intersect(float4 s, rt_vec3 ro, rt_vec3 rd) {
    SphereHit h; h.didHit = false; h.frontFace = false; h.dst = 0.f;
    rt_vec3 oc = rt_sub(f4xyz(s), ro);
    float a = rt_dot(rd, rd);
    float b = rt_dot(oc, rd);
    float c = rt_dot(oc, oc) - s.w * s.w;
    float disc = b * b - a * c;
    if (disc >= 0.f) {
        float sq = rt_sqrt(disc);
        float dst = (b - sq) / a;
        h.frontFace = true;
        if (dst < 0.f) {
            dst = (b + sq) / a;
            h.frontFace = false;
            if (dst < 0.f) return h;
        }
        h.didHit = true;
        h.dst = dst;
    }
    return h;
}

__device__ __forceinline__ float box_intersect(float4 lo, float4 hi, rt_vec3 ro, rt_vec3 inv);

__device__ __forceinline__ bool ray_is_plain(rt_vec3 wo, rt_vec3 wd) {
    const uint32_t E = 0x7f800000u, M = 0x7fffffffu;
    return ((rt_f2u(wd.x) & M) - 1u < E - 1u) && ((rt_f2u(wd.y) & M) - 1u < E - 1u) && ((rt_f2u(wd.z) & M) - 1u < E - 1u) &&
           ((rt_f2u(wo.x) & M) < E) && ((rt_f2u(wo.y) & M) < E) && ((rt_f2u(wo.z) & M) < E) &&
           rt_f2u(wo.x) != 0x80000000u && rt_f2u(wo.y) != 0x80000000u && rt_f2u(wo.z) != 0x80000000u;
}

__device__ __forceinline__ bool vec_is_plain(rt_vec3 v) {
    const uint32_t E = 0x7f800000u, M = 0x7fffffffu;
    return ((rt_f2u(v.x) & M) < E) && ((rt_f2u(v.y) & M) < E) && ((rt_f2u(v.z) & M) < E) &&
           rt_f2u(v.x) != 0x80000000u && rt_f2u(v.y) != 0x80000000u && rt_f2u(v.z) != 0x80000000u;
}

__device__ __forceinline__ bool origin_within(rt_vec3 o, float limit) {
    return rt_max(rt_max(rt_abs(o.x), rt_abs(o.y)), rt_abs(o.z)) <= limit;
}
__device__ __forceinline__ uint32_t reach_mask_from(const float4* boxes, uint32_t n, rt_vec3 ro, rt_vec3 rd, float originLimit) {
    uint32_t reach = 0xffffffffu;
    if (n && ray_is_plain(ro, rd) && origin_within(ro, originLimit)) {
        const rt_vec3 inv = rt_v3(1.f / rd.x, 1.f / rd.y, 1.f / rd.z);
// ... 225 lines not shown
                    }
                } else {
                    if (obj >= sc.objectCount) break;
                    float4 r0 = sc.objInv[3 * obj], r1 = sc.objInv[3 * obj + 1], r2 = sc.objInv[3 * obj + 2];
                    uint4 meta = sc.objMeta[obj];
                    trd = xform_dir_rows(r0, r1, r2, rd);
                    tro = xform_point_rows(r0, r1, r2, ro);
                    inv = rt_v3(1.f / trd.x, 1.f / trd.y, 1.f / trd.z);
                    curIdx = meta.x;
                    curCnt = meta.y;
                    if (curCnt) leaf_from_ref(sc, meta.x, curIdx, curCnt);
                    obj++;
                }
                have = true;
            }
            if (curCnt != 0) {
                nTri += curCnt;
                bool closer = false;
                for (uint32_t j = curIdx; j < curIdx + curCnt; j++) {
                    float4 a = sc.triPos[3 * j], b = sc.triPos[3 * j + 1], c = sc.triPos[3 * j + 2];
                    TriHit h = tri_intersect(tro, trd, f4xyz(a), f4xyz(b), f4xyz(c), __float_as_uint(a.w) != 0u);
                    if (h.didHit && h.dst < best) { best = h.dst; bestObj = obj - 1; bestTri = j; closer = true; }
                }
                have = false;
                if (closer && best < earlyT) { best = RT_MISS_DST; bestObj = RT_HIT_NONE; bestTri = 0; break; }
            } else {
                const float4* pr = sc.nodes + 2 * (size_t)curIdx;
                float4 lo1 = pr[0], hi1 = pr[1], lo2 = pr[2], hi2 = pr[3];
                float d1 = box_intersect(lo1, hi1, tro, inv);
                float d2 = box_intersect(lo2, hi2, tro, inv);
                nBox += 2;
                bool nearA = d1 <= d2;
                float dNear = nearA ? d1 : d2;
                float dFar = nearA ? d2 : d1;
                uint32_t nW = __float_as_uint(nearA ? lo1.w : lo2.w), nCnt = __float_as_uint(nearA ? hi1.w : hi2.w);
                uint32_t fW = __float_as_uint(nearA ? lo2.w : lo1.w);
                if (dFar < best) {
                    stack[sp * RT_WAVE] = fW;
                    sp++;
                }
                if (dNear < best) {
                    curIdx = nW; curCnt = nCnt;
                    if (nCnt) leaf_from_ref(sc, nW, curIdx, curCnt);
                } else have = false;
            }
        }

        ps.hit(kind)[slot] = make_float4(best, __uint_as_float(bestObj), __uint_as_float(bestTri), 0.f);
        if (kind == RAY_MAIN && ps.statBox()) { ps.statBox()[slot] += nBox; ps.statTri()[slot] += nTri; }
        if (ta.perRayBox) { ta.perRayBox[gid] = nBox; ta.perRayTri[gid] = nTri; }
        didHit = bestObj != RT_HIT_NONE;
    }

    unsigned long long wb = wave_sum_u64(nBox), wt = wave_sum_u64(nTri);
    uint32_t wr = wave_sum_u32(live ? 1u : 0u), wh = wave_sum_u32(didHit);
    if (lane_id() == 0) {
        atomicAdd(&ta.counters->boxTests, wb);
        atomicAdd(&ta.counters->triTests, wt);
        atomicAdd(&ta.counters->raysTraced, (unsigned long long)wr);
        atomicAdd(&ta.counters->raysHit, (unsigned long long)wh);
    }
}

#define RT_META_LDS 128u
#define RT_CUR_IDLE 0xffffffffu
#define RT_CUR_NEED 0xfffffffeu
#define RT_CUR_SETUP 0xfffffffdu
#define RT_CUR_WORLD 0xfffffffcu
#define RT_CUR_INIT 0xfffffffbu
#define RT_CUR_DONE 0xfffffffau
#define RT_CUR_LEAF_MAX 0xfffffff0u

struct TracePwArgs {
    const uint32_t* queue;
    const uint32_t* count;
    uint32_t* head;
    uint32_t refill;
    uint32_t chunk;
    uint32_t wSetup, wLeaf;
    uint32_t fastLanes;
    uint32_t fastShare;
    uint32_t* perRayBox;
    uint32_t* perRayTri;
    DevCounters* counters;
    unsigned long long* phaseStats;
    unsigned long long* waveTimes;
    uint32_t* overflow;
    const uint32_t* countAux;
    const uint32_t* countAux2;
    uint32_t auxOffset;
};

#define RT_STAMP_AFTER_LOADS(acc, t0) do { asm volatile("s_waitcnt vmcnt(0) lgkmcnt(0)" ::: "memory"); (acc) += clock64() - (t0); } while (0)

struct WaveTotals {
    uint32_t totBox = 0, totTri = 0, totRays = 0, totHits = 0;
    uint32_t totSkipBox = 0;
    uint32_t dbgRounds[4] = {0, 0, 0, 0}, dbgLanes[4] = {0, 0, 0, 0};
    unsigned long long dbgCycles[4] = {0, 0, 0, 0};
    unsigned long long dbgLoad[4] = {0, 0, 0, 0};
    uint32_t dbgWait[4] = {0, 0, 0, 0};
};

template <int STACK, bool OVF, bool PIX, bool STATS, bool LOCAL, bool CULL, int HOT = 0, bool ROOMY = false, bool ALPHA = false>
__device__ __forceinline__ void trace_wave(const DevScene& sc, const PathState& ps, const TracePwArgs& ta, uint32_t* stack, uint32_t* ovf,
                                           size_t ovfStride, const uint32_t* localList, uint32_t n, WaveTotals& wt, const uint2* metaLds,
                                           const float4* hotLds = nullptr) {
    uint32_t cur = RT_CUR_IDLE;
    uint32_t id = 0, qidx = 0;
    rt_vec3 trd = rt_v3(0, 0, 0);
    rt_f2 troXY = {0.f, 0.f}, invXY = {0.f, 0.f}, zOI = {0.f, 0.f};
    bool plain = false;
    bool atWorld = false;
    float best = RT_MISS_DST;
    uint32_t bestObj = RT_HIT_NONE, bestTri = 0;
    uint32_t obj = 0, sp = 0;
    uint32_t nxW = 0, nxFlags = 0;
    uint32_t rayBox = 0, rayTri = 0;
    bool exhausted = LOCAL;
    uint32_t resBase = 0, resCount = LOCAL ? n : 0u;
    uint32_t nextChunk = LOCAL ? 0u : min(ta.chunk, max(16u, n / (2u * gridDim.x * (RT_BLOCK / RT_WAVE))));

    uint32_t thr = ta.fastLanes;
    const uint32_t nMain = LOCAL ? 0u : *ta.count, nAux = (LOCAL || !ta.countAux) ? 0u : *ta.countAux;

    uint32_t reach = 0xffffffffu;
    float earlyT = 0.f;

    auto fetch_next_meta = [&]() {
        uint32_t skip = 0;
        if (CULL && obj - sc.maskBase < 32u) {
            const uint32_t w = obj - sc.maskBase;
            const uint32_t m = reach >> w;
            skip = m ? (uint32_t)__ffs((int)m) - 1u : 32u - w;
            if (skip) {
                const uint2 c0 = sc.objSkipCost[w], c1 = sc.objSkipCost[w + skip];
                if (PIX) { rayBox += c1.x - c0.x; rayTri += c1.y - c0.y; } else { wt.totBox += c1.x - c0.x; wt.totTri += c1.y - c0.y; }
                wt.totSkipBox += c1.x - c0.x;
            }
            obj += skip;
        }
        uint32_t fl = 0;
        if (obj < sc.objectCount) {
            if (obj < RT_META_LDS) {
                const uint2 m = metaLds[obj];
                nxW = m.x; fl = m.y;
            } else {
                const uint4 m = sc.objMeta[obj];
                nxW = m.x; fl = m.w & 0xffu;
            }
        }
        nxFlags = CULL ? (fl | (skip << 8)) : fl;
    };
    auto cur_object = [&]() { return CULL ? obj - 1u - (nxFlags >> 8) : obj - 1u; };

    for (;;) {
        const unsigned long long tRound = STATS ? clock64() : 0ull;
        int roundKind = 2;
        const unsigned long long mI = __ballot((int32_t)cur >= 0);
        uint32_t nI = __popcll(mI);
        bool runI = nI >= thr;
        if (!runI) {
            const unsigned long long mIdle = __ballot(cur == RT_CUR_IDLE);
            const uint32_t nIdle = __popcll(mIdle);
            if (nIdle == RT_WAVE && exhausted && resCount == 0) break;
            if (ta.fastShare) thr = min(ta.fastLanes, max(4u, ((RT_WAVE - nIdle) * ta.fastShare) >> 4));
            if (nIdle >= ta.refill && (resCount || !exhausted)) {
// ... 213 lines not shown
            }
        }

        {
            const bool need = cur == RT_CUR_NEED;
            const bool has = sp > 0;
            uint32_t top;
            if (OVF) {
                top = stack[min((has ? sp : 1u) - 1u, (uint32_t)STACK) * RT_WAVE];
                if (need && sp > (uint32_t)STACK) top = ((const RT_AS_GLOBAL uint32_t*)ovf)[(sp - 1u - STACK) * ovfStride];
            } else {
                top = stack[((has ? sp : 1u) - 1u) * RT_WAVE];
            }
            const bool objLeft = obj < sc.objectCount;
            const bool ident = (nxFlags & RT_OBJ_IDENTITY) && plain;
            const uint32_t whenEmpty = objLeft ? (ident ? (atWorld ? nxW : RT_CUR_WORLD) : RT_CUR_SETUP) : RT_CUR_DONE;
            const bool enter = need && !has && objLeft && ident && atWorld;
            cur = need ? (has ? top : whenEmpty) : cur;
            sp -= (need && has) ? 1u : 0u;
            if (enter) {
                obj++;
                fetch_next_meta();
            }
            if (cur == RT_CUR_DONE) {
                const uint32_t slot = id >> 2, kind = LOCAL ? (id & 3u) : ray_kind(id);
                ps.hit(kind)[slot] = make_float4(best, __uint_as_float(bestObj), __uint_as_float(bestTri), 0.f);
                if (PIX && kind == RAY_MAIN) { ps.statBox()[slot] += rayBox; ps.statTri()[slot] += rayTri; }
                if (PIX) {
                    if (ta.perRayBox) { ta.perRayBox[qidx] = rayBox; ta.perRayTri[qidx] = rayTri; }
                    wt.totBox += rayBox; wt.totTri += rayTri;
                }
                wt.totHits += (bestObj != RT_HIT_NONE) ? 1u : 0u;
                cur = RT_CUR_IDLE;
            }
        }
        if (STATS) wt.dbgCycles[roundKind] += clock64() - tRound;
    }

}

__device__ __forceinline__ void fill_meta_lds(const DevScene& sc, uint2* s_meta) {
    if (threadIdx.x < RT_META_LDS) {
        uint2 m = make_uint2(0u, 0u);
        if (threadIdx.x < sc.objectCount) { const uint4 q = sc.objMeta[threadIdx.x]; m = make_uint2(q.x, q.w & 0xffu); }
        s_meta[threadIdx.x] = m;
    }
    __syncthreads();
}

template <int STACK, bool OVF, bool PIX, bool STATS, bool CULL, int HOT, bool ROOMY, bool ALPHA>
__device__ __forceinline__ void trace_pw_block(const DevScene& sc, const PathState& ps, const TracePwArgs& ta) {
    __shared__ uint32_t s_stack[(RT_BLOCK / RT_WAVE) * (STACK + 1) * RT_WAVE];
    __shared__ uint2 s_meta[RT_META_LDS];
    __shared__ float4 s_hot[HOT ? 4 * HOT : 1];
    if (HOT) for (uint32_t k = threadIdx.x; k < 2u * min(sc.hotNodes, 2u * (uint32_t)HOT); k += RT_BLOCK) s_hot[k] = sc.nodesPk[k];
    fill_meta_lds(sc, s_meta);
    uint32_t* stack = s_stack + (threadIdx.x / RT_WAVE) * (STACK + 1) * RT_WAVE + (threadIdx.x & (RT_WAVE - 1));
    uint32_t* ovf = OVF ? ta.overflow + (size_t)blockIdx.x * RT_BLOCK + threadIdx.x : nullptr;
    const size_t ovfStride = (size_t)gridDim.x * RT_BLOCK;
    WaveTotals wt;
    const unsigned long long tStart = STATS ? wall_clock64() : 0ull;
    trace_wave<STACK, OVF, PIX, STATS, false, CULL, HOT, ROOMY, ALPHA>(sc, ps, ta, stack, ovf, ovfStride, nullptr, *ta.count + (ta.countAux ? *ta.countAux + *ta.countAux2 : 0u), wt, s_meta, s_hot);

    const uint32_t skipTrips = STATS ? wave_sum_u32(wt.dbgWait[3]) : 0u;
    if (STATS && lane_id() == 0) {
        const size_t w = (size_t)blockIdx.x * (RT_BLOCK / RT_WAVE) + threadIdx.x / RT_WAVE;
        if (ta.waveTimes) {
            ta.waveTimes[2 * w] = tStart;
            ta.waveTimes[2 * w + 1] = wall_clock64();
        }
        for (int k = 0; k < 4; k++) {
            atomicAdd(&ta.phaseStats[k], (unsigned long long)wt.dbgRounds[k]);
            atomicAdd(&ta.phaseStats[4 + k], (unsigned long long)wt.dbgLanes[k]);
            atomicAdd(&ta.phaseStats[8 + k], wt.dbgCycles[k]);
            atomicAdd(&ta.phaseStats[16 + k], wt.dbgLoad[k]);
            if (k < 3) atomicAdd(&ta.phaseStats[12 + k], (unsigned long long)wt.dbgWait[k]);
            else atomicAdd(&ta.phaseStats[20], (unsigned long long)skipTrips);
        }
    }
    unsigned long long wb = wave_sum_u64(wt.totBox), wtri = wave_sum_u64(wt.totTri);
    uint32_t wr = wave_sum_u32(wt.totRays), wh = wave_sum_u32(wt.totHits);
    const unsigned long long wskip = CULL ? wave_sum_u64(wt.totSkipBox) : 0ull;
    if (lane_id() == 0 && wr) {
        if (CULL && wskip) atomicAdd(&ta.counters->skippedBoxTests, wskip);
        atomicAdd(&ta.counters->boxTests, wb);
        atomicAdd(&ta.counters->triTests, wtri);
        atomicAdd(&ta.counters->raysTraced, (unsigned long long)wr);
        atomicAdd(&ta.counters->raysHit, (unsigned long long)wh);
    }
}

template <int STACK, bool OVF, bool PIX, bool STATS, bool CULL, int HOT = 0, int BLOCKS = 6>
__global__ __launch_bounds__(RT_BLOCK, BLOCKS) void k_trace_pw(DevScene sc, PathState ps, TracePwArgs ta) {
    trace_pw_block<STACK, OVF, PIX, STATS, CULL, HOT, BLOCKS == 5, false>(sc, ps, ta);
}
template <bool PIX>
__global__ __launch_bounds__(RT_BLOCK, 4) void k_trace_pw_alpha(DevScene sc, PathState ps, TracePwArgs ta) {
    trace_pw_block<24, true, PIX, false, true, 0, true, true>(sc, ps, ta);
}

struct FullHit {
    rt_vec3 hitPoint, normal;
    uint32_t materialIndex;
    bool frontFace;
    float u, v;
};

__device__ __forceinline__ rt_vec3 albedo_texel(const DevScene& sc, uint32_t slot, uint32_t tri, uint32_t obj, rt_vec3 ro, rt_vec3 rd) {
    float bu, bv, bw;
    {
        const float4 i0 = rt_global(sc.objInv)[3 * obj], i1 = rt_global(sc.objInv)[3 * obj + 1], i2 = rt_global(sc.objInv)[3 * obj + 2];
        const float4 p0 = rt_global(sc.triPos)[3 * (size_t)tri], p1 = rt_global(sc.triPos)[3 * (size_t)tri + 1], p2 = rt_global(sc.triPos)[3 * (size_t)tri + 2];
        const TriHit h = tri_intersect(xform_point_rows(i0, i1, i2, ro), xform_dir_rows(i0, i1, i2, rd), f4xyz(p0), f4xyz(p1), f4xyz(p2), __float_as_uint(p0.w) != 0u);
        bu = h.u; bv = h.v; bw = h.w;
    }
    const float4 a = rt_global(sc.triUV)[2 * (size_t)tri], b = rt_global(sc.triUV)[2 * (size_t)tri + 1];
    float u = (bw * a.x + bu * a.z) + bv * b.x, v = (bw * a.y + bu * a.w) + bv * b.y;
    const bool e01 = a.x == a.z && a.y == a.w, e12 = a.z == b.x && a.w == b.y, e20 = b.x == a.x && b.y == a.y;
    if (e01 || e12 || e20) { u = 0.5f; v = 0.5f; }
    const uint4 ti = rt_global(sc.texInfo)[slot];
    const bool clampEdge = ((rt_global(sc.objMeta)[obj].w >> RT_OBJ_SAMPLER_SHIFT) & RT_OBJ_SAMPLER_MASK) == 1u;
    const uint32_t x = rt_tex_index(u, ti.y, clampEdge), y = rt_tex_index(1.f - v, ti.z, clampEdge);
    const uint32_t t = rt_global(sc.texels)[(size_t)ti.x + (size_t)y * ti.y + x];
    return rt_v3(rt_srgb8_to_linear(t & 0xffu), rt_srgb8_to_linear((t >> 8) & 0xffu), rt_srgb8_to_linear((t >> 16) & 0xffu));
}

template <bool MAPS = false>
__device__ __forceinline__ FullHit reconstruct_hit(const DevScene& sc, rt_vec3 ro, rt_vec3 rd, uint32_t obj, uint32_t tri) {
    FullHit f;
    f.u = 0.f; f.v = 0.f;
    if (obj & RT_HIT_SPHERE) {
        uint32_t i = obj & ~RT_HIT_SPHERE;
        float4 s = rt_global(sc.spheres)[i];
        SphereHit h = sphere_intersect(s, ro, rd);
        f.hitPoint = rt_add(ro, rt_scale(rd, h.dst));
        f.normal = rt_scale(rt_normalize(rt_sub(f.hitPoint, f4xyz(s))), h.frontFace ? 1.f : -1.f);
        f.materialIndex = rt_global(sc.sphereMat)[i];
        f.frontFace = h.frontFace;
        return f;
    }
    const uint4 meta = rt_global(sc.objMeta)[obj];
    const bool ident = RT_SHADE_IDENT && (meta.w & RT_OBJ_FWD_IDENTITY) && ray_is_plain(ro, rd);
    rt_vec3 trd = rd, tro = ro;
    if (!ident) {
        const float4* inv = rt_global(sc.objInv) + 3 * obj;
        const float4 i0 = inv[0], i1 = inv[1], i2 = inv[2];
        trd = xform_dir_rows(i0, i1, i2, rd);
        tro = xform_point_rows(i0, i1, i2, ro);
    }
    const float4* tp = rt_global(sc.triPos) + 3 * (size_t)tri;
    float4 a = tp[0], b = tp[1], c = tp[2];
    TriHit h = tri_intersect(tro, trd, f4xyz(a), f4xyz(b), f4xyz(c), __float_as_uint(a.w) != 0u);
    const float4* tn = rt_global(sc.triNrm) + 3 * (size_t)tri;
    rt_vec3 n0 = f4xyz(tn[0]), n1 = f4xyz(tn[1]), n2 = f4xyz(tn[2]);
    rt_vec3 ni = rt_add(rt_add(rt_scale(n0, h.w), rt_scale(n1, h.u)), rt_scale(n2, h.v));
    if (MAPS) {
        const HitUV q = hit_uv(sc, tri, h.u, h.v, h.w);
        f.u = q.u; f.v = q.v;
        const uint32_t bumpSlot = __float_as_uint(rt_global(sc.mats)[3 * meta.z + 2].w);
        if (bumpSlot < sc.texCount) {
            const bool clampEdge = ((meta.w >> RT_OBJ_SAMPLER_SHIFT) & RT_OBJ_SAMPLER_MASK) == 1u;
            const float h0 = rt_srgb8_to_linear(map_red8(sc, bumpSlot, clampEdge, q.u, q.v, false, false));
            const float hx = rt_srgb8_to_linear(map_red8(sc, bumpSlot, clampEdge, q.u, q.v, true, false)) - h0;
            const float hy = rt_srgb8_to_linear(map_red8(sc, bumpSlot, clampEdge, q.u, q.v, false, true)) - h0;
            ni = rt_bump_normal(ni, rt_sub(f4xyz(b), f4xyz(a)), rt_sub(f4xyz(c), f4xyz(a)), q.du1, q.dv1, q.du2, q.dv2, hx, hy);
        }
    }
    ni = rt_scale(ni, h.frontFace ? 1.f : -1.f);
    rt_vec3 op = rt_add(tro, rt_scale(trd, h.dst));
    if (ident && vec_is_plain(ni) && vec_is_plain(op)) {
        f.normal = rt_normalize(ni);
// ... 35 lines not shown

__device__ __forceinline__ float light_cos(rt_vec3 dir) { return rt_dot(rt_v3(0.f, -1.f, 0.f), dir); }
__device__ __forceinline__ float light_sample_pdf(const DevScene& sc, float t, uint32_t obj, float cosTheta) {
    if (obj == RT_HIT_NONE) return 0.f;
    uint32_t m = hit_material(sc, obj);
    if (rt_global(sc.mats)[3 * m + 1].w == 0.f) return 0.f;
    float sq = t * t;
    return sq / (cosTheta * 0.4444444f);
}

__device__ __forceinline__ rt_vec3 primary_dir(const FrameParams& fp, uint32_t gx, uint32_t gy) {
    float u = (float)gx / (float)fp.width;
    float v = (float)gy / (float)fp.height;
    rt_vec3 point = rt_add(rt_v3(fp.bottomLeft[0], fp.bottomLeft[1], fp.bottomLeft[2]),
                           rt_v3(fp.planeWidth * u, fp.planeHeight * v, 0.f));
    rt_vec3 dir = rt_normalize(point);
    return rt_xform_point(fp.camRot, dir);
}

__device__ __forceinline__ uint32_t slot_frame(const FrameParams& fp, uint32_t slot) { return (slot >> 6) % fp.nFrames; }
__device__ __forceinline__ uint32_t slot_in_tile(const FrameParams& fp, uint32_t slot) { return ((slot >> 6) / fp.nFrames << 6) | (slot & 63u); }
__device__ __forceinline__ uint32_t frame_slot(const FrameParams& fp, uint32_t frame, uint32_t tileSlot) {
    return ((tileSlot >> 6) * fp.nFrames + frame) * 64u + (tileSlot & 63u);
}

__device__ __forceinline__ void slot_to_pixel(const FrameParams& fp, uint32_t slot, uint32_t& gx, uint32_t& gy, uint32_t& k) {
    if (fp.nFrames > 1u) slot = slot_in_tile(fp, slot);
    const uint32_t tiledSlots = fp.tiled ? (fp.nRows & ~7u) * fp.width : 0u;
    if (slot < tiledSlots) {
        const uint32_t tile = slot >> 6, in = slot & 63u;
        const uint32_t tilesPerRow = fp.width >> 3;
        const uint32_t tyb = tile / tilesPerRow, txb = tile - tyb * tilesPerRow;
        gx = (txb << 3) + (in & 7u);
        k = (tyb << 3) + (in >> 3);
    } else {
        k = slot / fp.width;
        gx = slot - k * fp.width;
    }
    gy = fp.row0 + k * fp.rowStride;
}

__device__ __forceinline__ void init_path(const DevScene& sc, const PathState& ps, const FrameParams& fp, uint32_t slot) {
    uint32_t gx, gy;
    uint32_t krow;
    slot_to_pixel(fp, slot, gx, gy, krow);
    ps.rayO()[slot] = make_float4(fp.camPos[0], fp.camPos[1], fp.camPos[2], 1.f);
    const rt_vec3 pd = primary_dir(fp, gx, gy);
    uint32_t startingSeed = fp.startingSeed;
    if (fp.nFrames > 1u) {
        uint32_t lol = fp.frameCount + slot_frame(fp, slot);
        startingSeed = (uint32_t)(rt_random(&lol) * 23892183.f);
    }
    ps.rayD()[slot] = mk4u(pd, gy * fp.width + gx + startingSeed);
    ps.camDir()[slot] = mk4(pd, 0.f);
    ps.hit(RAY_MAIN)[slot] = sphere_seed(sc, rt_v3(fp.camPos[0], fp.camPos[1], fp.camPos[2]), pd);
    ps.att()[slot] = make_float4(1.f, 1.f, 1.f, __uint_as_float(0u));
    ps.total()[slot] = make_float4(0.f, 0.f, 0.f, __uint_as_float(0u));
    ps.accum()[slot] = make_float4(0.f, 0.f, 0.f, 0.f);
    ps.statBox()[slot] = 0;
    ps.statTri()[slot] = 0;
}

#define RT_QUEUE_HOLE 0xffffffffu
__global__ __launch_bounds__(RT_BLOCK) void k_raygen(DevScene sc, PathState ps, uint32_t* activeOut, uint32_t* raysOut, FrameParams fp,
                                                     uint32_t slotBegin, uint32_t slotEnd) {
    const uint32_t pos = blockIdx.x * RT_BLOCK + threadIdx.x;
    const uint32_t slot = slotBegin + pos;
    if (slot >= slotEnd) return;
    if (fp.nFrames > 1u && slot_in_tile(fp, slot) >= fp.nPixels) {
        activeOut[pos] = RT_QUEUE_HOLE;
        raysOut[pos] = RT_QUEUE_HOLE;
        return;
    }
    init_path(sc, ps, fp, slot);
    activeOut[pos] = slot;
    raysOut[pos] = slot << 2;
}

struct ShadeArgs {
    const uint32_t* inActive;
    const uint32_t* inCount;
    uint32_t* outActive;
    uint32_t* outRays;
    uint32_t* outActiveCount;
    uint32_t* outRayCount;
    ShadeStatStripe* stats;
    uint32_t* outAuxCount;
    uint32_t* outAuxCount2;
    uint32_t auxOffset;
};

template <bool MAPS = false, bool QUEUED = false>
__device__ __forceinline__ void shade_path(const DevScene& sc, const PathState& ps, const FrameParams& fp, uint32_t slot, bool& alive,
                                           uint32_t& auxMask, uint32_t& refRays, uint32_t& nPaths, uint32_t& emitTests, bool withMask = true) {
    bool wantAux = false;
    auxMask = 0;
    rt_vec3 auxOrigin = rt_v3(0, 0, 0), auxL = auxOrigin, auxC = auxOrigin;
    rt_vec3 auxAlbedo = auxOrigin;
    float auxNdotL = 0.f, auxCosPdfL = 0.f, auxCosPdfC = 0.f;
    float auxCosL = 0.f, auxCosC = 0.f;
    const float4 sO = ps.rayO()[slot], sD = ps.rayD()[slot], sA = ps.att()[slot], sT = ps.total()[slot];
    const float4 hM = (QUEUED && fp.camReuse && (__float_as_uint(sA.w) & 0x0fffffffu) == 0u && __float_as_uint(sT.w) != 0u) ? ps.camHit()[slot]
                                                                                                                        : ps.hit(RAY_MAIN)[slot];
    rt_vec3 ro = f4xyz(sO), rd = f4xyz(sD);
    rt_vec3 att = f4xyz(sA), total = f4xyz(sT);
    float misW = sO.w;
    uint32_t state = __float_as_uint(sD.w);
    uint32_t jraw = __float_as_uint(sA.w);
    uint32_t samplesDone = __float_as_uint(sT.w);
    uint32_t j = jraw & 0x0fffffffu;
    const bool pending = (jraw >> 31) != 0u;
    rt_vec3 direct = (jraw & 0x40000000u) ? rt_v3(-1.f, -1.f, -1.f) : rt_v3(0.f, 0.f, 0.f);
    bool specular = false;

    const uint32_t obj = __float_as_uint(hM.y);
    const uint32_t hitTriIdx = __float_as_uint(hM.z);
    refRays = 1;
    if (fp.camReuse && j == 0u && samplesDone == 0u) ps.camHit()[slot] = hM;

    bool done = false;
    bool zeroed = false;

    if (obj != RT_HIT_NONE) {
        if (pending) {
            float4 hL = make_float4(RT_MISS_DST, __uint_as_float(RT_HIT_NONE), 0.f, 0.f), hC = hL;
            if (!(jraw & 0x20000000u)) hL = ps.hit(RAY_NEE)[slot];
            if (!(jraw & 0x10000000u)) hC = ps.hit(RAY_PROBE)[slot];
            const float4 pM = ps.pendMis()[slot];
            float tL = hL.x, tC = hC.x;
            uint32_t oL = __float_as_uint(hL.y), oC = __float_as_uint(hC.y);
            uint32_t lm = (oL == RT_HIT_NONE) ? 0u : hit_material(sc, oL);
            float4 lmE = rt_global(sc.mats)[3 * lm + 1];
            float realLightPDF = light_sample_pdf(sc, tL, oL, pM.x);
            float cosinePDF = pM.z;
            float misWeight1 = realLightPDF * realLightPDF / (realLightPDF * realLightPDF + cosinePDF * cosinePDF);
            if (rt_isnan(misWeight1)) misWeight1 = 0.f;
            float lightPDF = light_sample_pdf(sc, tC, oC, pM.y);
            float realCosinePDF = pM.w;
            float misWeight2 = realCosinePDF * realCosinePDF / (lightPDF * lightPDF + realCosinePDF * realCosinePDF);
            if (rt_isnan(misWeight2)) misWeight2 = 0.f;
            const float4 pA = ps.pendAlbedo()[slot];
            rt_vec3 albedo = f4xyz(pA);
            rt_vec3 dl = rt_scale(rt_v3(lmE.x, lmE.y, lmE.z), lmE.w);
            float k = (realLightPDF == 0.f) ? 0.f : misWeight1 / realLightPDF;
            rt_vec3 f = rt_scale(rt_scale(rt_scale(albedo, RT_INV_PI), pA.w), k);
            direct = rt_mul(dl, f);
            misW = misWeight2;
        }

        FullHit hit = reconstruct_hit<MAPS>(sc, ro, rd, obj, hitTriIdx);
        const float4* mp = rt_global(sc.mats) + 3 * hit.materialIndex;
        float4 mA = mp[0], mE = mp[1], mI = mp[2];
        if (MAPS) {
            const uint32_t metalSlot = __float_as_uint(mI.z);
            if (metalSlot < sc.texCount && !(obj & RT_HIT_SPHERE))
                mA.w = rt_srgb8_to_linear(map_red8(sc, metalSlot, ((rt_global(sc.objMeta)[obj].w >> RT_OBJ_SAMPLER_SHIFT) & RT_OBJ_SAMPLER_MASK) == 1u, hit.u, hit.v, false, false));
        }

        rt_vec3 emission = rt_scale(rt_v3(mE.x, mE.y, mE.z), mE.w);
        emission = rt_v3(emission.x / misW, emission.y / misW, emission.z / misW);
        rt_vec3 finalLight = direct.x == -1.f ? emission : direct;
        total = rt_add(total, rt_mul(finalLight, att));
        if (j == 0) total = rt_add(total, emission);
        if (rt_isnan(total.x) || rt_isnan(total.y) || rt_isnan(total.z) || total.x < 0.f || total.y < 0.f || total.z < 0.f) {
            done = true;
            zeroed = true;
        } else {
            rt_vec3 sampledDir, radiance;
            float originSign = 1.f;
            bool diffuse = false;
            if (mA.w != 0.f) {
                sampledDir = rt_reflect(rd, hit.normal);
                radiance = rt_v3(1.f, 1.f, 1.f);
// ... 58 lines not shown
                ro = rt_add(hit.hitPoint, rt_scale(rt_scale(hit.normal, originSign), 0.00001f));
                rd = sampledDir;
                j++;
                if (j > fp.bounceLimit) done = true;
                else wantAux = diffuse;
            }
        }
    } else {
        total = rt_add(total, rt_mul(att, environment_light(fp.env, rd)));
        done = true;
    }

    if (done) {
        nPaths = 1;
        float4 acc = ps.accum()[slot];
        if (zeroed) total = rt_v3(0.f, 0.f, 0.f);
        const rt_vec3 sum = rt_add(f4xyz(acc), total);
        ps.accum()[slot] = mk4(sum, 0.f);
        samplesDone++;
        if (samplesDone < fp.samples) {
            ro = rt_v3(fp.camPos[0], fp.camPos[1], fp.camPos[2]);
            rd = f4xyz(ps.camDir()[slot]);
            att = rt_v3(1.f, 1.f, 1.f);
            total = rt_v3(0.f, 0.f, 0.f);
            specular = false;
            misW = 1.f;
            j = 0;
            alive = true;
            wantAux = false;
        }
    } else {
        alive = true;
    }

    if (alive) {
        if (done && fp.camReuse) {
            if (!QUEUED) ps.hit(RAY_MAIN)[slot] = ps.camHit()[slot];
            auxMask |= 4u;
        } else {
            const float4 seed = sphere_seed(sc, ro, rd, withMask);
            if (QUEUED && seed_is_blank(seed)) auxMask |= 8u;
            else ps.hit(RAY_MAIN)[slot] = seed;
        }
        if (wantAux) {
            float4 sL = sphere_seed(sc, auxOrigin, auxL, withMask), sC = sphere_seed(sc, auxOrigin, auxC, withMask);
            auxMask |= 3u;
            if (sc.emitMode) {
                float tL, tC;
                emitter_min_t2(sc, auxOrigin, auxL, auxC, tL, tC, emitTests);
                if (!(tL < RT_MISS_DST) || sL.x < tL) { sL.x = RT_MISS_DST; sL.y = __uint_as_float(RT_HIT_NONE); auxMask &= ~1u; }
                else sL.w = tL;
                if (!(tC < RT_MISS_DST) || sC.x < tC) { sC.x = RT_MISS_DST; sC.y = __uint_as_float(RT_HIT_NONE); auxMask &= ~2u; }
                else sC.w = tC;
            }
            const bool albedoFinite = !(rt_isnan(auxAlbedo.x) || rt_isnan(auxAlbedo.y) || rt_isnan(auxAlbedo.z) || rt_isinf(auxAlbedo.x) || rt_isinf(auxAlbedo.y) || rt_isinf(auxAlbedo.z));
            if ((auxMask & 3u) == 0u && albedoFinite) {
                float m2 = auxCosPdfC * auxCosPdfC / (0.f * 0.f + auxCosPdfC * auxCosPdfC);
                if (rt_isnan(m2)) m2 = 0.f;
                misW = m2;
                wantAux = false;
            } else {
                if (auxMask & 1u) ps.hit(RAY_NEE)[slot] = sL;
                if (auxMask & 2u) ps.hit(RAY_PROBE)[slot] = sC;
                if (auxMask & 3u) ps.auxO()[slot] = mk4(auxOrigin, 0.f);
                if (auxMask & 1u) ps.auxDL()[slot] = mk4(auxL, 0.f);
                if (auxMask & 2u) ps.auxDC()[slot] = mk4(auxC, 0.f);
                ps.pendAlbedo()[slot] = mk4(auxAlbedo, auxNdotL);
                ps.pendMis()[slot] = make_float4(auxCosL, auxCosC, auxCosPdfL, auxCosPdfC);
            }
        }
        const uint32_t answered = wantAux ? (((auxMask & 1u) ? 0u : 0x20000000u) | ((auxMask & 2u) ? 0u : 0x10000000u)) : 0u;
        ps.rayO()[slot] = mk4(ro, misW);
        ps.rayD()[slot] = mk4u(rd, state);
        ps.att()[slot] = mk4u(att, j | (wantAux ? 0x80000000u : 0u) | (specular ? 0x40000000u : 0u) | answered);
        const float4 nT = mk4u(total, samplesDone);
        if (!QUEUED || __float_as_uint(nT.x) != __float_as_uint(sT.x) || __float_as_uint(nT.y) != __float_as_uint(sT.y) ||
            __float_as_uint(nT.z) != __float_as_uint(sT.z) || __float_as_uint(nT.w) != __float_as_uint(sT.w))
            ps.total()[slot] = nT;
    }
}

template <bool MAPS>
__device__ __forceinline__ void shade_block(const DevScene& sc, const PathState& ps, const ShadeArgs& sa, const FrameParams& fp) {
    __shared__ uint32_t s_cnt[RT_BLOCK / RT_WAVE][8];
    __shared__ uint32_t s_base[4];
    const uint32_t n = *sa.inCount;
    if (blockIdx.x * RT_BLOCK >= n) return;
    const uint32_t gid = blockIdx.x * RT_BLOCK + threadIdx.x;
    const bool live = gid < n;

    bool alive = false;
    uint32_t auxMask = 0;
    uint32_t slot = 0;
    uint32_t refRays = 0, nPaths = 0, emitTests = 0;
    bool path = live;
    if (live) {
        slot = sa.inActive[gid];
        path = slot != 0xffffffffu;
        if (path) shade_path<MAPS, true>(sc, ps, fp, slot, alive, auxMask, refRays, nPaths, emitTests);
    }

    const unsigned long long mAlive = __ballot(alive), mM = __ballot(alive && !(auxMask & 4u));
    const unsigned long long mL = __ballot(alive && (auxMask & 1u)), mC = __ballot(alive && (auxMask & 2u));
    const uint32_t nAlive = __popcll(mAlive), nM = __popcll(mM), nL = __popcll(mL), nC = __popcll(mC);
    const uint32_t wRef = wave_sum_u32(refRays), wPaths = wave_sum_u32(nPaths), wSeg = wave_sum_u32(path ? 1u : 0u), wEmit = wave_sum_u32(emitTests);
    const uint32_t wv = threadIdx.x / RT_WAVE;
    if (lane_id() == 0) {
        s_cnt[wv][0] = nAlive; s_cnt[wv][1] = nM; s_cnt[wv][2] = wRef; s_cnt[wv][3] = wPaths; s_cnt[wv][4] = wSeg; s_cnt[wv][5] = wEmit; s_cnt[wv][6] = nL; s_cnt[wv][7] = nC;
    }
    __syncthreads();
    if (threadIdx.x == 0) {
        uint32_t tA = 0, tR = 0, tRef = 0, tP = 0, tS = 0, tE = 0, tX = 0, tY = 0;
        for (int w = 0; w < RT_BLOCK / RT_WAVE; w++) { tA += s_cnt[w][0]; tR += s_cnt[w][1]; tRef += s_cnt[w][2]; tP += s_cnt[w][3]; tS += s_cnt[w][4]; tE += s_cnt[w][5]; tX += s_cnt[w][6]; tY += s_cnt[w][7]; }
        s_base[0] = tA ? atomicAdd(sa.outActiveCount, tA) : 0u;
        s_base[1] = tR ? atomicAdd(sa.outRayCount, tR) : 0u;
        s_base[2] = tX ? atomicAdd(RT_QUEUE_ORDER ? sa.outAuxCount2 : sa.outAuxCount, tX) : 0u;
        s_base[3] = tY ? atomicAdd(RT_QUEUE_ORDER ? sa.outAuxCount : sa.outAuxCount2, tY) : 0u;
        ShadeStatStripe* const st = sa.stats + (blockIdx.x & (RT_STAT_STRIPES - 1u));
        atomicAdd(&st->raysReference, (unsigned long long)tRef);
        if (tP) atomicAdd(&st->paths, (unsigned long long)tP);
        atomicAdd(&st->segments, (unsigned long long)tS);
        if (tE) atomicAdd(&st->emitterTests, (unsigned long long)tE);
    }
    __syncthreads();
    if (alive) {
        uint32_t baseA = s_base[0], baseR = s_base[1];
        uint32_t baseX = (RT_QUEUE_ORDER ? 2u : 1u) * sa.auxOffset + s_base[2], baseY = (RT_QUEUE_ORDER ? 1u : 2u) * sa.auxOffset + s_base[3];
        for (uint32_t w = 0; w < wv; w++) { baseA += s_cnt[w][0]; baseR += s_cnt[w][1]; baseX += s_cnt[w][6]; baseY += s_cnt[w][7]; }
        sa.outActive[baseA + lanes_below(mAlive)] = slot;
        if (!(auxMask & 4u)) sa.outRays[baseR + lanes_below(mM)] = (slot << 2) | ((auxMask & 8u) ? RAY_MAIN_BLANK : (uint32_t)RAY_MAIN);
        if (auxMask & 1u) sa.outRays[baseX + lanes_below(mL)] = (slot << 2) | RAY_NEE;
        if (auxMask & 2u) sa.outRays[baseY + lanes_below(mC)] = (slot << 2) | RAY_PROBE;
    }
}

__global__ __launch_bounds__(RT_BLOCK) void k_shade(DevScene sc, PathState ps, ShadeArgs sa, FrameParams fp) { shade_block<false>(sc, ps, sa, fp); }
__global__ __launch_bounds__(RT_BLOCK) void k_shade_maps(DevScene sc, PathState ps, ShadeArgs sa, FrameParams fp) { shade_block<true>(sc, ps, sa, fp); }

__device__ __forceinline__ rt_vec3 blend_frame(const FrameParams& fp, uint32_t frameCount, float4 oldc, float4 accum) {
    rt_vec3 out = f4xyz(accum);
    float fs = (float)fp.samples;
    out = rt_v3(out.x / fs, out.y / fs, out.z / fs);
    float weight = 1.f / ((float)frameCount + 1.f);
    rt_vec3 blended = rt_add(rt_scale(rt_v3(oldc.x, oldc.y, oldc.z), 1.f - weight), rt_scale(out, weight));
    rt_vec3 fin = fp.progressive ? blended : out;
    if (rt_isnan(fin.x) || rt_isnan(fin.y) || rt_isnan(fin.z) || rt_isinf(fin.x) || rt_isinf(fin.y) || rt_isinf(fin.z))
        fin = rt_v3(1.f, 0.f, 1.f);
    return fin;
}

__device__ __forceinline__ void resolve_pixel(const PathState& ps, const FrameParams& fp, float4* rgba, uint32_t slot) {
    uint32_t gx, gy, krow;
    slot_to_pixel(fp, slot, gx, gy, krow);
    const size_t px = (size_t)krow * fp.width + gx;
    rt_vec3 fin = blend_frame(fp, fp.frameCount, rgba[px], ps.accum()[slot]);
    float s0 = (float)ps.statBox()[slot], s1 = (float)ps.statTri()[slot];
    float boxCap = (float)fp.boxCap, triCap = (float)fp.triCap;
    if (fp.debug == 0) {
        fin = s0 > boxCap ? rt_v3(1.f, 0.f, 0.f) : rt_v3(s0 / boxCap, s0 / boxCap, s0 / boxCap);
    } else if (fp.debug == 1) {
        fin = s1 > triCap ? rt_v3(1.f, 0.f, 0.f) : rt_v3(s1 / triCap, s1 / triCap, s1 / triCap);
    } else if (fp.debug == 2) {
        fin = rt_v3(s0 / boxCap, 0.f, s1 / triCap);
    }
    rgba[px] = make_float4(fin.x, fin.y, fin.z, 1.f);
}

__global__ __launch_bounds__(RT_BLOCK) void k_blend_frames(PathState ps, FrameParams fp, float4* rgba) {
    const uint32_t slot = blockIdx.x * RT_BLOCK + threadIdx.x;
    if (slot >= fp.nPixels) return;
    uint32_t gx, gy, krow;
    slot_to_pixel(fp, frame_slot(fp, 0u, slot), gx, gy, krow);
    const size_t px = (size_t)krow * fp.width + gx;
    float4 c = rgba[px];
    for (uint32_t f = 0; f < fp.nFrames; f++) {
        const rt_vec3 fin = blend_frame(fp, fp.frameCount + f, c, ps.accum()[frame_slot(fp, f, slot)]);
        c = make_float4(fin.x, fin.y, fin.z, 1.f);
    }
    rgba[px] = c;
}

__global__ __launch_bounds__(RT_BLOCK) void k_resolve(PathState ps, FrameParams fp, float4* rgba) {
    uint32_t slot = blockIdx.x * RT_BLOCK + threadIdx.x;
    if (slot >= fp.nPixels) return;
    resolve_pixel(ps, fp, rgba, slot);
}

struct FusedArgs {
    uint32_t* batchHead;
    float4* rgba;
    DevCounters* counters;
    uint32_t* overflow;
    uint32_t refill, wSetup, wLeaf, fastLanes;
    uint32_t batchPixels;
    uint32_t scatter;
    uint32_t fastShare;
    unsigned long long* waveTimes;
    uint32_t pixelRefill;
};

template <typename T>
__device__ __forceinline__ const T* opaque_kernarg() {
    unsigned long long v = (unsigned long long)__builtin_amdgcn_kernarg_segment_ptr();
    asm volatile("" : "+s"(v));
    return (const T*)(const RT_AS_CONSTANT T*)v;
}

struct FusedKernArgs {
    DevScene sc;
    PathState ps;
    FrameParams fp;
    FusedArgs fa;
};

template <int STACK, bool OVF, bool PIX, bool CULL>
__global__ __launch_bounds__(RT_BLOCK, 5) void k_render_fused(FusedKernArgs ka) {
    constexpr bool ALPHA = false, MAPS = false;
#include "rt_fused_body.hip.inc"
}
template <bool PIX>
// ... 113 lines not shown
__global__ __launch_bounds__(RT_DN_BLOCK) void k_dn_variance(DenoiseFrame f, const float4* work, float4* out) {
    uint32_t x, y;
    if (!dn_pixel(f, x, y)) return;
    const size_t p = (size_t)y * f.width + x;
    const float4 e = work[p];
    if (e.w < 0.f) { out[p] = e; return; }
    const uint32_t x0 = x >= 2u ? x - 2u : 0u, x1 = x + 2u < f.width ? x + 2u : f.width - 1u;
    const uint32_t y0 = y >= 2u ? y - 2u : 0u, y1 = y + 2u < f.height ? y + 2u : f.height - 1u;
    float sum = 0.f, n = 0.f;
    for (uint32_t qy = y0; qy <= y1; qy++)
        for (uint32_t qx = x0; qx <= x1; qx++) {
            const float4 q = work[(size_t)qy * f.width + qx];
            if (q.w >= 0.f) { sum += dn_luminance(q); n += 1.f; }
        }
    const float mu = sum / n;
    float ss = 0.f;
    for (uint32_t qy = y0; qy <= y1; qy++)
        for (uint32_t qx = x0; qx <= x1; qx++) {
            const float4 q = work[(size_t)qy * f.width + qx];
            if (q.w >= 0.f) { const float d = dn_luminance(q) - mu; ss += d * d; }
        }
    const float z = f.normalDepth[p].w;
    auto diff = [&](bool hasF, size_t qf, bool hasB, size_t qb) {
        hasF = hasF && work[qf].w >= 0.f;
        hasB = hasB && work[qb].w >= 0.f;
        const float fd = hasF ? f.normalDepth[qf].w - z : 0.f, bd = hasB ? z - f.normalDepth[qb].w : 0.f;
        return hasF && hasB ? (rt_abs(bd) < rt_abs(fd) ? bd : fd) : hasF ? fd : bd;
    };
    f.grad[p] = make_float2(diff(x + 1u < f.width, p + 1, x > 0u, p - 1), diff(y + 1u < f.height, p + f.width, y > 0u, p - f.width));
    out[p] = make_float4(e.x, e.y, e.z, ss / n);
}

template <bool LAST>
__global__ __launch_bounds__(RT_DN_BLOCK) void k_dn_atrous(DenoiseFrame f, const float4* in, float4* out, float4* rgbaOut, int step,
                                                           float sigmaL, float sigmaN, float sigmaZ) {
    uint32_t x, y;
    if (!dn_pixel(f, x, y)) return;
    const size_t p = (size_t)y * f.width + x;
    const float4 c = in[p];
    if (c.w < 0.f) {
        if (LAST) rgbaOut[p] = f.rgba[p];
        else out[p] = c;
        return;
    }
    const float4 ndp = f.normalDepth[p];
    const float2 g = f.grad[p];
    const rt_vec3 np = f4xyz(ndp);
    const float lp = dn_luminance(c), lumDen = sigmaL * rt_sqrt(c.w) + 1e-4f, zEps = 1e-4f * ndp.w;
    float sw = 0.f, sv = 0.f;
    rt_vec3 se = rt_v3(0.f, 0.f, 0.f);
#pragma unroll
    for (int j = -2; j <= 2; j++) {
        const int qy = (int)y + step * j;
        if (qy < 0 || qy >= (int)f.height) continue;
#pragma unroll
        for (int i = -2; i <= 2; i++) {
            const int qx = (int)x + step * i;
            if (qx < 0 || qx >= (int)f.width) continue;
            const size_t q = (size_t)qy * f.width + (uint32_t)qx;
            const float4 e = in[q];
            if (e.w < 0.f) continue;
            const float4 ndq = f.normalDepth[q];
            float w = dn_h(i) * dn_h(j);
            if (sigmaN != 0.f) w = w * rt_pow(rt_max(0.f, rt_dot(np, f4xyz(ndq))), sigmaN);
            const float dz = rt_abs(ndp.w - ndq.w);
            const float az = dz == 0.f ? 0.f : dz / (sigmaZ * rt_abs(g.x * (float)(step * i) + g.y * (float)(step * j)) + zEps);
            const float al = rt_abs(lp - dn_luminance(e)) / lumDen;
            w = w * rt_exp2(-(az + al) * 1.44269504088896341f);
            sw += w;
            se = rt_add(se, rt_scale(f4xyz(e), w));
            sv += (w * w) * e.w;
        }
    }
    const rt_vec3 ep = rt_v3(se.x / sw, se.y / sw, se.z / sw);
    if (LAST) {
        const float4 a = f.albedo[p];
        rgbaOut[p] = make_float4(ep.x * rt_max(a.x, 1e-3f), ep.y * rt_max(a.y, 1e-3f), ep.z * rt_max(a.z, 1e-3f), f.rgba[p].w);
    } else {
        out[p] = mk4(ep, sv / (sw * sw));
    }
}

__global__ void k_init_counts(uint32_t* counts, uint32_t n) {
    if (threadIdx.x == 0) { counts[0] = n; counts[1] = 0; counts[2] = n; counts[3] = 0; counts[4] = 0; counts[5] = 0; counts[6] = 0; counts[7] = 0; counts[8] = 0; }
}
__global__ __launch_bounds__(RT_STAT_STRIPES) void k_fold_shade_stats(ShadeStatStripe* stats, DevCounters* counters) {
    ShadeStatStripe* const st = stats + threadIdx.x;
    const unsigned long long a = wave_sum_u64(st->raysReference), b = wave_sum_u64(st->paths), c = wave_sum_u64(st->segments), d = wave_sum_u64(st->emitterTests);
    st->raysReference = 0; st->paths = 0; st->segments = 0; st->emitterTests = 0;
    if (lane_id() == 0) {
        atomicAdd(&counters->raysReference, a);
        atomicAdd(&counters->paths, b);
        atomicAdd(&counters->segments, c);
        atomicAdd(&counters->emitterTests, d);
    }
}
__global__ void k_zero_counts(uint32_t* a, uint32_t* b, uint32_t* c, uint32_t* d, uint32_t* e) {
    if (threadIdx.x == 0) { *a = 0; *b = 0; *c = 0; *d = 0; *e = 0; }
}

__device__ __host__ inline uint32_t selftest_mix(uint32_t h, float v) {
    h ^= rt_f2u(v);
    h *= 16777619u;
    return h;
}
__device__ __host__ inline uint32_t selftest_one(float a, float b) {
    uint32_t h = 2166136261u;
    float s, c;
    rt_sincos(a * 6.2831855f, &s, &c);
    h = selftest_mix(h, s); h = selftest_mix(h, c);
    h = selftest_mix(h, a / b); h = selftest_mix(h, 1.f / (b + 0.25f));
    h = selftest_mix(h, rt_sqrt(a)); h = selftest_mix(h, rt_pow(a, 5.f)); h = selftest_mix(h, rt_pow(a, 0.35f));
    h = selftest_mix(h, rt_log2(b + 1e-3f)); h = selftest_mix(h, rt_exp2(a * 20.f - 10.f));
    rt_vec3 v = rt_normalize(rt_v3(a - 0.5f, b - 0.5f, a * b + 0.1f));
    h = selftest_mix(h, v.x); h = selftest_mix(h, v.y); h = selftest_mix(h, v.z);
    h = selftest_mix(h, rt_dot(v, rt_v3(b, a, 0.3f)));
    rt_vec3 r = rt_refract(v, rt_normalize(rt_v3(0.1f, 1.f, b)), 0.5f + a);
    h = selftest_mix(h, r.x); h = selftest_mix(h, r.y); h = selftest_mix(h, r.z);
    h = selftest_mix(h, rt_smoothstep(0.f, 0.4f, a)); h = selftest_mix(h, rt_min(a, b)); h = selftest_mix(h, rt_max(a, b));
    h = selftest_mix(h, a * b + b);
    uint32_t st = rt_f2u(a) ^ (rt_f2u(b) * 7u);
    h = selftest_mix(h, rt_random(&st));
    return h;
}
__global__ void k_selftest(const float* a, const float* b, uint32_t n, uint32_t* hashOut, uint32_t* bitsOut, const float* kat) {
    uint32_t i = blockIdx.x * blockDim.x + threadIdx.x;
    if (i < n) hashOut[i] = selftest_one(a[i], b[i]);
    if (i == 0) *bitsOut = rt_selftest_bits(kat);
}

__global__ __launch_bounds__(RT_BLOCK) void k_deinterleave_rows(const float4* __restrict__ strips, float4* __restrict__ frame, uint32_t width,
                                                                uint32_t height, uint32_t nRanks) {
    const size_t i = (size_t)blockIdx.x * RT_BLOCK + threadIdx.x;
    if (i >= (size_t)width * height) return;
    const uint32_t y = (uint32_t)(i / width), x = (uint32_t)(i - (size_t)y * width);
    const uint32_t r = y % nRanks, k = y / nRanks;
    const uint32_t full = height / nRanks, extra = height % nRanks;
    const size_t before = (size_t)r * full + (r < extra ? r : extra);
    frame[i] = strips[(before + k) * width + x];
}

__global__ void k_math_probe(const float* in, float* out, uint32_t n) {
    const uint32_t i = blockIdx.x * blockDim.x + threadIdx.x;
    if (i >= n) return;
    float a[32], o[64];
    for (int k = 0; k < 32; k++) a[k] = in[(size_t)i * 32 + k];
    rt_math_probe(a, o);
    for (int k = 0; k < 64; k++) out[(size_t)i * 64 + k] = o[k];
}

__global__ void k_copy_f4(const float4* __restrict__ src, float4* __restrict__ dst, size_t n) {
    size_t i = (size_t)blockIdx.x * blockDim.x + threadIdx.x;
    size_t stride = (size_t)gridDim.x * blockDim.x;
    for (; i < n; i += stride) dst[i] = src[i];
}
```

Before: 4426 Mrays/s.

## Stripe trace stats atomics, pack queue counters, and group shade blocks over multiple tiles

Trace kernel statistics now go to per-CU striped stat buffers instead of one global DevCounters, and are folded by a follow-up kernel. This removes contention on a few global atomics. Queue counters are re-laid out so the active/main and aux pairs sit next to each other and can each be reserved with one 64-bit atomic. The shade kernel can also process up to four block-tiles per block when the launch is large, which cuts the number of block-level atomics, and it adds a launch-bounds occupancy hint. The trade-off is more complex scan logic in the shade kernel, plus an extra shared-memory prefix pass that runs serially over rows.

```diff
diff --git a/ray_tracer_amd/csrc/rt_device.hip b/ray_tracer_amd/csrc/rt_device.hip
--- a/ray_tracer_amd/csrc/rt_device.hip
+++ b/ray_tracer_amd/csrc/rt_device.hip
@@ -70,6 +70,8 @@
     DevBuf waveTimeBuf;
     DevBuf aovBuf, aovCounterBuf;
     DevBuf shadeStatBuf;
+    DevBuf traceStatBuf;
+    uint32_t shadeGroupMin[2] = {0, 0};
     uint32_t aovPixels = 0; bool aovValid = false;
     RowsOf fbRows, aovRows;
     DevBuf dnWorkBuf, dnHostBuf, dnOutBuf;
@@ -111,6 +113,7 @@
         int batchFixed = 80;
         int fusedMaps = 0;
         int probe = 1;
+        int shadeGroup = 0;
     } tune;
 
     struct Measured {
@@ -350,12 +353,12 @@
     const uint32_t blocks = std::max(1u, std::min((nBatches + (RT_BLOCK / RT_WAVE) - 1) / (RT_BLOCK / RT_WAVE), resident));
     uint32_t* overflow;
     if ((rc = overflow_buf(c, d, k.stack, k.ovf, resident, &overflow))) return rc;
-    RT_HIP(c, hipMemsetAsync(d.counts + 5, 0, 4, d.stream));
+    RT_HIP(c, hipMemsetAsync(d.counts + RT_CNT_FUSED_WORK, 0, 4, d.stream));
     const uint32_t fastLanes = c->tune.fastLanesSet ? (uint32_t)c->tune.fastLanes : (c->meas.boxPerRay >= (double)c->tune.fusedBelowBoxTests ? 40u : 24u);
     const uint32_t wLeaf = (uint32_t)c->tune.wLeafFused;
     unsigned long long* waveTimes = nullptr;
     if (d.phaseStats && (rc = wave_time_buf(c, blocks, &waveTimes))) return rc;
-    FusedArgs fa{d.counts + 5, fb, (DevCounters*)c->counterBuf.p, overflow, (uint32_t)c->tune.refill, (uint32_t)c->tune.wSetupFused, wLeaf, fastLanes, batchPixels, g, (uint32_t)c->tune.fastShare, waveTimes, pixelRefill};
+    FusedArgs fa{d.counts + RT_CNT_FUSED_WORK, fb, (DevCounters*)c->counterBuf.p, overflow, (uint32_t)c->tune.refill, (uint32_t)c->tune.wSetupFused, wLeaf, fastLanes, batchPixels, g, (uint32_t)c->tune.fastShare, waveTimes, pixelRefill};
     const FusedKernArgs ka{d.sc, c->ps, fp, fa};
     memcpy(c->rep.lastKernel, k.name, sizeof k.name);
     hipLaunchKernelGGL(k.kernel, dim3(blocks), dim3(RT_BLOCK), 0, d.stream, ka);
@@ -401,13 +404,17 @@
         const bool longRays = c->meas.boxPerRay >= (double)c->tune.fusedBelowBoxTests;
         const uint32_t refillMk = c->tune.refillMkSet ? (uint32_t)c->tune.refillMk : (longRays ? 12u : 16u);
         const uint32_t wSetup = c->tune.wSetupSet ? (uint32_t)c->tune.wSetup : (longRays ? 32u : 16u);
-        const TracePwArgs pa{ta.queue, ta.count, d.counts + 4, refillMk, (uint32_t)c->tune.chunk, wSetup, (uint32_t)c->tune.wLeaf, (uint32_t)c->tune.fastLanes, (uint32_t)c->tune.fastShare,
-                             ta.perRayBox, ta.perRayTri, ta.counters, (unsigned long long*)((char*)c->counterBuf.p + sizeof(DevCounters)), waveTimes, overflow, ta.countAux, ta.countAux2, ta.auxOffset};
+        const TracePwArgs pa{ta.queue, ta.count, d.counts + RT_CNT_WORK, refillMk, (uint32_t)c->tune.chunk, wSetup, (uint32_t)c->tune.wLeaf, (uint32_t)c->tune.fastLanes, (uint32_t)c->tune.fastShare,
+                             ta.perRayBox, ta.perRayTri, (TraceStatStripe*)c->traceStatBuf.p, (unsigned long long*)((char*)c->counterBuf.p + sizeof(DevCounters)), waveTimes, overflow, ta.countAux, ta.countAux2, ta.auxOffset};
         memcpy(c->rep.lastKernel, k.name, sizeof k.name);
         hipLaunchKernelGGL(k.kernel, dim3(blocks), dim3(RT_BLOCK), 0, d.stream, d.sc, c->ps, pa);
     }
     RT_HIP(c, hipGetLastError());
     return prof_end(c, d, ev);
+}
+
+void fold_trace_stats(rt_ctx* c, DevCounters* counters) {
+    hipLaunchKernelGGL(k_fold_shade_stats, dim3(1), dim3(RT_STAT_STRIPES), 0, c->stream, (ShadeStatStripe*)nullptr, (TraceStatStripe*)c->traceStatBuf.p, counters);
 }
 
 void poll_ray_cost(rt_ctx* c) {
@@ -553,6 +560,8 @@
     (void)hipMemsetAsync(c->aovCounterBuf.p, 0, sizeof(DevCounters), c->stream);
     if (dev_alloc(c, c->shadeStatBuf, sizeof(ShadeStatStripe) * RT_STAT_STRIPES) != 0) { rt_destroy(c); return -7; }
     (void)hipMemsetAsync(c->shadeStatBuf.p, 0, sizeof(ShadeStatStripe) * RT_STAT_STRIPES, c->stream);
+    if (dev_alloc(c, c->traceStatBuf, sizeof(TraceStatStripe) * RT_STAT_STRIPES) != 0) { rt_destroy(c); return -7; }
+    (void)hipMemsetAsync(c->traceStatBuf.p, 0, sizeof(TraceStatStripe) * RT_STAT_STRIPES, c->stream);
     (void)hipStreamSynchronize(c->stream);
     *out = c;
     return 0;
@@ -727,6 +736,16 @@
     return nLanes;
 }
 
+uint32_t shade_group_min(rt_ctx* c, bool maps) {
+    uint32_t& cached = c->shadeGroupMin[maps ? 1 : 0];
+    if (!cached) {
+        int perCU = 0;
+        if (hipOccupancyMaxActiveBlocksPerMultiprocessor(&perCU, maps ? k_shade_maps : k_shade, RT_BLOCK, 0) != hipSuccess || perCU <= 0) perCU = 4;
+        cached = 2u * RT_SHADE_GROUP * RT_BLOCK * (uint32_t)perCU * (uint32_t)c->numCUs;
+    }
+    return cached;
+}
+
 struct Lane { Dispatch d; hipEvent_t poll; uint32_t begin, n, ubActive; int cur; bool pollPending, done; };
 void slice_parts(rt_ctx* c, const Dispatch& d, uint32_t nSlots, uint32_t nFrames, int nLanes, Lane* lane) {
     const uint32_t unit = 256u * std::max(1u, nFrames);
@@ -736,7 +755,7 @@
         const uint32_t u = units / (uint32_t)nLanes + ((uint32_t)l < units % (uint32_t)nLanes ? 1u : 0u);
         const uint32_t end = std::min(nSlots, at + u * unit);
         lane[l] = Lane{d, l ? c->pollEventSide[l - 1] : c->pollEvent, at, end - at, end - at, 0, false, end == at};
-        lane[l].d.stream = l ? c->sideStream[l - 1] : c->stream; lane[l].d.counts = c->q.counts + 16 * l; lane[l].d.part = l;
+        lane[l].d.stream = l ? c->sideStream[l - 1] : c->stream; lane[l].d.counts = c->q.counts + RT_CNT_WORDS * l; lane[l].d.part = l;
         at = end;
     }
     const int gridPct = part_grid_pct(c->tune, nLanes, lane[0].n);
@@ -745,6 +764,8 @@
 
 int render_rounds(rt_ctx* c, const FrameParams& fp, Lane* lane, int nLanes) {
     DevCounters* dc = (DevCounters*)c->counterBuf.p;
+    const bool shadeMaps = (lane[0].d.sc.mapFlags & (RT_MAP_METALNESS | RT_MAP_BUMP)) != 0u;
+    const uint32_t groupMin = shade_group_min(c, shadeMaps);
     int rc = 0;
     if (nLanes > 1) {
         RT_HIP(c, hipEventRecord(c->forkEvent, c->stream));
@@ -761,12 +782,12 @@
             const int cur = L.cur, nxt = cur ^ 1;
             uint32_t* const active[2] = {c->q.active[0] + L.begin, c->q.active[1] + L.begin};
             uint32_t* const rays[2] = {c->q.rays[0] + 3 * (size_t)L.begin, c->q.rays[1] + 3 * (size_t)L.begin};
-            hipLaunchKernelGGL(k_zero_counts, dim3(1), dim3(64), 0, stream, counts + nxt, counts + 2 + nxt, counts + 4, counts + 5 + nxt, counts + 7 + nxt);
-            TraceArgs ta{rays[cur], counts + 2 + cur, nullptr, nullptr, dc, counts + 5 + cur, counts + 7 + cur, L.n};
+            hipLaunchKernelGGL(k_zero_counts, dim3(1), dim3(64), 0, stream, counts, (uint32_t)nxt);
+            TraceArgs ta{rays[cur], counts + RT_CNT_MAIN(cur), nullptr, nullptr, dc, counts + RT_CNT_AUX(cur), counts + RT_CNT_AUX2(cur), L.n};
             const uint64_t ubRays = std::min<uint64_t>((uint64_t)L.ubActive * 3, (uint64_t)L.n * 3);
             if ((rc = launch_trace(c, L.d, (uint32_t)ubRays, ta))) break;
-            ShadeArgs sa{active[cur], counts + cur, active[nxt], rays[nxt], counts + nxt, counts + 2 + nxt, (ShadeStatStripe*)c->shadeStatBuf.p, counts + 5 + nxt, counts + 7 + nxt, L.n};
-            if (L.d.sc.mapFlags & (RT_MAP_METALNESS | RT_MAP_BUMP)) hipLaunchKernelGGL(k_shade_maps, dim3((L.ubActive + RT_BLOCK - 1) / RT_BLOCK), dim3(RT_BLOCK), 0, stream, L.d.sc, c->ps, sa, fp);
+            ShadeArgs sa{active[cur], counts + RT_CNT_ACTIVE(cur), active[nxt], rays[nxt], counts + RT_CNT_ACTIVE(nxt), (ShadeStatStripe*)c->shadeStatBuf.p, L.n, (uint32_t)c->tune.shadeGroup, groupMin};
+            if (shadeMaps) hipLaunchKernelGGL(k_shade_maps, dim3((L.ubActive + RT_BLOCK - 1) / RT_BLOCK), dim3(RT_BLOCK), 0, stream, L.d.sc, c->ps, sa, fp);
             else hipLaunchKernelGGL(k_shade, dim3((L.ubActive + RT_BLOCK - 1) / RT_BLOCK), dim3(RT_BLOCK), 0, stream, L.d.sc, c->ps, sa, fp);
             L.cur = nxt;
             if (L.pollPending && hipEventQuery(L.poll) == hipSuccess) {
@@ -775,7 +796,7 @@
                 if (L.ubActive == 0) { L.done = true; continue; }
             }
             if (!L.pollPending && (it & 7u) == 7u) {
-                if (hipMemcpyAsync(c->hostCounts + 8 + l, counts + L.cur, 4, hipMemcpyDeviceToHost, stream) == hipSuccess &&
+                if (hipMemcpyAsync(c->hostCounts + 8 + l, counts + RT_CNT_ACTIVE(L.cur), 4, hipMemcpyDeviceToHost, stream) == hipSuccess &&
                     hipEventRecord(L.poll, stream) == hipSuccess)
                     L.pollPending = true;
             }
@@ -786,7 +807,7 @@
         RT_HIP(c, hipEventRecord(c->joinEvent[l - 1], lane[l].d.stream));
         RT_HIP(c, hipStreamWaitEvent(c->stream, c->joinEvent[l - 1], 0));
     }
-    hipLaunchKernelGGL(k_fold_shade_stats, dim3(1), dim3(RT_STAT_STRIPES), 0, c->stream, (ShadeStatStripe*)c->shadeStatBuf.p, dc);
+    hipLaunchKernelGGL(k_fold_shade_stats, dim3(1), dim3(RT_STAT_STRIPES), 0, c->stream, (ShadeStatStripe*)c->shadeStatBuf.p, (TraceStatStripe*)c->traceStatBuf.p, dc);
     return rc;
 }
 
@@ -983,13 +1004,14 @@
     uint32_t* prb = (uint32_t*)c->scratchBuf.p;
     uint32_t* prt = prb + n;
     RtHit* dh = (RtHit*)((char*)c->scratchBuf.p + (((size_t)n * 8 + 255) & ~(size_t)255));
-    c->hostCounts[0] = n; c->hostCounts[1] = 0; c->hostCounts[2] = 0; c->hostCounts[3] = 0; c->hostCounts[4] = 0;
-    RT_HIP(c, hipMemcpyAsync(c->q.counts, c->hostCounts, 20, hipMemcpyHostToDevice, c->stream));
+    hipLaunchKernelGGL(k_init_counts, dim3(1), dim3(64), 0, c->stream, c->q.counts, n);
     RT_HIP(c, hipMemsetAsync(c->ps.statBox(), 0, (size_t)n * 4, c->stream));
     RT_HIP(c, hipMemsetAsync(c->ps.statTri(), 0, (size_t)n * 4, c->stream));
     hipLaunchKernelGGL(k_seed_rays, dim3((n + RT_BLOCK - 1) / RT_BLOCK), dim3(RT_BLOCK), 0, c->stream, c->sc, c->ps, n);
-    TraceArgs ta{nullptr, c->q.counts, prb, prt, (DevCounters*)c->counterBuf.p};
-    if ((rc = launch_trace(c, one_part(c, c->sc, false), n, ta))) return rc;
+    TraceArgs ta{nullptr, c->q.counts + RT_CNT_MAIN(0u), prb, prt, (DevCounters*)c->counterBuf.p};
+    rc = launch_trace(c, one_part(c, c->sc, false), n, ta);
+    fold_trace_stats(c, ta.counters);
+    if (rc) return rc;
     hipLaunchKernelGGL(k_hit_details, dim3((n + RT_BLOCK - 1) / RT_BLOCK), dim3(RT_BLOCK), 0, c->stream, c->sc, c->ps, n, prb, prt, dh);
     RT_HIP(c, hipGetLastError());
     RT_HIP(c, hipMemcpyAsync(hitsOut, dh, (size_t)n * sizeof(RtHit), hipMemcpyDeviceToHost, c->stream));
@@ -1028,8 +1050,10 @@
     hipLaunchKernelGGL(k_aov_rays, dim3(blocks), dim3(RT_BLOCK), 0, c->stream, d.sc, c->ps, fp);
     hipLaunchKernelGGL(k_init_counts, dim3(1), dim3(64), 0, c->stream, c->q.counts, nPixels);
     RT_HIP(c, hipGetLastError());
-    const TraceArgs ta{nullptr, c->q.counts, nullptr, nullptr, (DevCounters*)c->aovCounterBuf.p};
-    if ((rc = launch_trace(c, d, nPixels, ta))) return rc;
+    const TraceArgs ta{nullptr, c->q.counts + RT_CNT_MAIN(0u), nullptr, nullptr, (DevCounters*)c->aovCounterBuf.p};
+    rc = launch_trace(c, d, nPixels, ta);
+    fold_trace_stats(c, ta.counters);
+    if (rc) return rc;
     hipLaunchKernelGGL(k_aov_resolve, dim3(blocks), dim3(RT_BLOCK), 0, c->stream, d.sc, c->ps, fp, out);
     RT_HIP(c, hipGetLastError());
     return 0;
@@ -1289,6 +1313,7 @@
     std::string k(key);
     if (k == "pipeline") { if (value < -1 || value > 1) return c->fail("pipeline: -1 (auto), 0 or 1"); c->tune.pipeline = value; }
     else if (k == "probe") { c->tune.probe = value ? 1 : 0; }
+    else if (k == "shade_group") { if (value != 0 && value != 1 && value != (int)RT_SHADE_GROUP) return c->fail("shade_group: 0 (by the launch's size), 1 or 4"); c->tune.shadeGroup = value; }
     else if (k == "frames_max_mslots") { if (value < 1 || value > 1000) return c->fail("frames_max_mslots: 1..1000 (millions of paths per multi-frame dispatch)"); c->tune.framesMaxSlots = (uint64_t)value << 20; }
     else if (k == "frames_per_launch") { if (value < 0) return c->fail("frames_per_launch >= 0"); c->tune.framesPerLaunch = value; }
     else if (k == "camera_reuse") { c->tune.cameraReuse = value ? 1 : 0; }
diff --git a/ray_tracer_amd/csrc/rt_fused_body.hip.inc b/ray_tracer_amd/csrc/rt_fused_body.hip.inc
--- a/ray_tracer_amd/csrc/rt_fused_body.hip.inc
+++ b/ray_tracer_amd/csrc/rt_fused_body.hip.inc
@@ -15,7 +15,7 @@
     uint32_t* list = s_list[wv];
     uint32_t* ovf = OVF ? fa.overflow + (size_t)blockIdx.x * RT_BLOCK + threadIdx.x : nullptr;
     const size_t ovfStride = (size_t)gridDim.x * RT_BLOCK;
-    const TracePwArgs ta{nullptr, nullptr, nullptr, fa.refill, 0u, fa.wSetup, fa.wLeaf, fa.fastLanes, fa.fastShare, nullptr, nullptr, fa.counters, nullptr, nullptr, fa.overflow};
+    const TracePwArgs ta{nullptr, nullptr, nullptr, fa.refill, 0u, fa.wSetup, fa.wLeaf, fa.fastLanes, fa.fastShare, nullptr, nullptr, (TraceStatStripe*)fa.counters, nullptr, nullptr, fa.overflow};
     WaveTotals wt;
     uint32_t refTot = 0, pathTot = 0, segTot = 0, emitTot = 0;
     const unsigned long long tKernelStart = fa.waveTimes ? wall_clock64() : 0ull;
diff --git a/ray_tracer_amd/csrc/rt_kernels.hip.h b/ray_tracer_amd/csrc/rt_kernels.hip.h
--- a/ray_tracer_amd/csrc/rt_kernels.hip.h
+++ b/ray_tracer_amd/csrc/rt_kernels.hip.h
@@ -124,6 +124,18 @@
     unsigned long long raysReference, paths, segments, emitterTests;
     unsigned long long pad[12];
 };
+struct TraceStatStripe {
+    unsigned long long boxTests, triTests, raysTraced, raysHit, skippedBoxTests;
+    unsigned long long pad[11];
+};
+
+#define RT_CNT_WORDS 16u
+#define RT_CNT_ACTIVE(p) (4u * (p))
+#define RT_CNT_MAIN(p) (4u * (p) + 1u)
+#define RT_CNT_AUX(p) (4u * (p) + 2u)
+#define RT_CNT_AUX2(p) (4u * (p) + 3u)
+#define RT_CNT_WORK 8u
+#define RT_CNT_FUSED_WORK 9u
 
 #define RT_AS_CONSTANT __attribute__((address_space(4)))
 #define RT_AS_GLOBAL __attribute__((address_space(1)))
@@ -515,7 +527,7 @@
     uint32_t fastShare;
     uint32_t* perRayBox;
     uint32_t* perRayTri;
-    DevCounters* counters;
+    TraceStatStripe* stats;
     unsigned long long* phaseStats;
     unsigned long long* waveTimes;
     uint32_t* overflow;
@@ -895,11 +907,13 @@
     uint32_t wr = wave_sum_u32(wt.totRays), wh = wave_sum_u32(wt.totHits);
     const unsigned long long wskip = CULL ? wave_sum_u64(wt.totSkipBox) : 0ull;
     if (lane_id() == 0 && wr) {
-        if (CULL && wskip) atomicAdd(&ta.counters->skippedBoxTests, wskip);
-        atomicAdd(&ta.counters->boxTests, wb);
-        atomicAdd(&ta.counters->triTests, wtri);
-        atomicAdd(&ta.counters->raysTraced, (unsigned long long)wr);
-        atomicAdd(&ta.counters->raysHit, (unsigned long long)wh);
+        const uint32_t cu = __smid();
+        TraceStatStripe* const st = ta.stats + ((cu ^ (cu >> 8)) & (RT_STAT_STRIPES - 1u));
+        if (CULL && wskip) atomicAdd(&st->skippedBoxTests, wskip);
+        atomicAdd(&st->boxTests, wb);
+        atomicAdd(&st->triTests, wtri);
+        atomicAdd(&st->raysTraced, (unsigned long long)wr);
+        atomicAdd(&st->raysHit, (unsigned long long)wh);
     }
 }
 
@@ -1101,13 +1115,13 @@
     const uint32_t* inCount;
     uint32_t* outActive;
     uint32_t* outRays;
-    uint32_t* outActiveCount;
-    uint32_t* outRayCount;
+    uint32_t* outCounts;
     ShadeStatStripe* stats;
-    uint32_t* outAuxCount;
-    uint32_t* outAuxCount2;
     uint32_t auxOffset;
+    uint32_t group;
+    uint32_t groupMin;
 };
+#define RT_SHADE_GROUP 4u
 
 template <bool MAPS = false, bool QUEUED = false>
 __device__ __forceinline__ void shade_path(const DevScene& sc, const PathState& ps, const FrameParams& fp, uint32_t slot, bool& alive,
@@ -1332,60 +1346,84 @@
 
 template <bool MAPS>
 __device__ __forceinline__ void shade_block(const DevScene& sc, const PathState& ps, const ShadeArgs& sa, const FrameParams& fp) {
-    __shared__ uint32_t s_cnt[RT_BLOCK / RT_WAVE][8];
-    __shared__ uint32_t s_base[4];
+    __shared__ uint32_t s_cnt[RT_SHADE_GROUP * (RT_BLOCK / RT_WAVE)][8];
     const uint32_t n = *sa.inCount;
-    if (blockIdx.x * RT_BLOCK >= n) return;
-    const uint32_t gid = blockIdx.x * RT_BLOCK + threadIdx.x;
-    const bool live = gid < n;
-
-    bool alive = false;
-    uint32_t auxMask = 0;
-    uint32_t slot = 0;
-    uint32_t refRays = 0, nPaths = 0, emitTests = 0;
-    bool path = live;
-    if (live) {
-        slot = sa.inActive[gid];
-        path = slot != 0xffffffffu;
-        if (path) shade_path<MAPS, true>(sc, ps, fp, slot, alive, auxMask, refRays, nPaths, emitTests);
-    }
-
-    const unsigned long long mAlive = __ballot(alive), mM = __ballot(alive && !(auxMask & 4u));
-    const unsigned long long mL = __ballot(alive && (auxMask & 1u)), mC = __ballot(alive && (auxMask & 2u));
-    const uint32_t nAlive = __popcll(mAlive), nM = __popcll(mM), nL = __popcll(mL), nC = __popcll(mC);
-    const uint32_t wRef = wave_sum_u32(refRays), wPaths = wave_sum_u32(nPaths), wSeg = wave_sum_u32(path ? 1u : 0u), wEmit = wave_sum_u32(emitTests);
+    const uint32_t K = sa.group ? sa.group : (n >= sa.groupMin ? RT_SHADE_GROUP : 1u);
+    const uint32_t first = blockIdx.x * K * RT_BLOCK;
+    if (first >= n) return;
+    const uint32_t iters = min(K, (n - first + RT_BLOCK - 1u) / RT_BLOCK);
     const uint32_t wv = threadIdx.x / RT_WAVE;
-    if (lane_id() == 0) {
-        s_cnt[wv][0] = nAlive; s_cnt[wv][1] = nM; s_cnt[wv][2] = wRef; s_cnt[wv][3] = wPaths; s_cnt[wv][4] = wSeg; s_cnt[wv][5] = wEmit; s_cnt[wv][6] = nL; s_cnt[wv][7] = nC;
-    }
+
+    uint32_t kept = 0;
+#pragma unroll 1
+    for (uint32_t i = 0; i < iters; i++) {
+        const uint32_t gid = first + i * RT_BLOCK + threadIdx.x;
+        bool alive = false;
+        uint32_t auxMask = 0;
+        uint32_t refRays = 0, nPaths = 0, emitTests = 0;
+        bool path = gid < n;
+        if (path) {
+            const uint32_t slot = sa.inActive[gid];
+            path = slot != 0xffffffffu;
+            if (path) shade_path<MAPS, true>(sc, ps, fp, slot, alive, auxMask, refRays, nPaths, emitTests);
+        }
+        const uint32_t nAlive = __popcll(__ballot(alive)), nM = __popcll(__ballot(alive && !(auxMask & 4u)));
+        const uint32_t nL = __popcll(__ballot(alive && (auxMask & 1u))), nC = __popcll(__ballot(alive && (auxMask & 2u)));
+        const uint32_t wRef = wave_sum_u32(refRays), wPaths = wave_sum_u32(nPaths), wSeg = wave_sum_u32(path ? 1u : 0u), wEmit = wave_sum_u32(emitTests);
+        if (lane_id() == 0) {
+            uint32_t* const row = s_cnt[i * (RT_BLOCK / RT_WAVE) + wv];
+            row[0] = nAlive; row[1] = nM; row[2] = wRef; row[3] = wPaths; row[4] = wSeg; row[5] = wEmit; row[6] = nL; row[7] = nC;
+        }
+        kept |= ((alive ? 16u : 0u) | (auxMask & 15u)) << (5u * i);
+    }
+
     __syncthreads();
-    if (threadIdx.x == 0) {
-        uint32_t tA = 0, tR = 0, tRef = 0, tP = 0, tS = 0, tE = 0, tX = 0, tY = 0;
-        for (int w = 0; w < RT_BLOCK / RT_WAVE; w++) { tA += s_cnt[w][0]; tR += s_cnt[w][1]; tRef += s_cnt[w][2]; tP += s_cnt[w][3]; tS += s_cnt[w][4]; tE += s_cnt[w][5]; tX += s_cnt[w][6]; tY += s_cnt[w][7]; }
-        s_base[0] = tA ? atomicAdd(sa.outActiveCount, tA) : 0u;
-        s_base[1] = tR ? atomicAdd(sa.outRayCount, tR) : 0u;
-        s_base[2] = tX ? atomicAdd(RT_QUEUE_ORDER ? sa.outAuxCount2 : sa.outAuxCount, tX) : 0u;
-        s_base[3] = tY ? atomicAdd(RT_QUEUE_ORDER ? sa.outAuxCount : sa.outAuxCount2, tY) : 0u;
-        ShadeStatStripe* const st = sa.stats + (blockIdx.x & (RT_STAT_STRIPES - 1u));
-        atomicAdd(&st->raysReference, (unsigned long long)tRef);
-        if (tP) atomicAdd(&st->paths, (unsigned long long)tP);
-        atomicAdd(&st->segments, (unsigned long long)tS);
-        if (tE) atomicAdd(&st->emitterTests, (unsigned long long)tE);
+    if (wv == 0) {
+        const uint32_t rows = iters * (RT_BLOCK / RT_WAVE), col = lane_id() & 7u;
+        uint32_t t = 0;
+        if (lane_id() < 8u) for (uint32_t r = 0; r < rows; r++) t += s_cnt[r][col];
+        const uint32_t tA = __builtin_amdgcn_readlane(t, 0), tR = __builtin_amdgcn_readlane(t, 1), tRef = __builtin_amdgcn_readlane(t, 2), tP = __builtin_amdgcn_readlane(t, 3);
+        const uint32_t tS = __builtin_amdgcn_readlane(t, 4), tE = __builtin_amdgcn_readlane(t, 5), tL = __builtin_amdgcn_readlane(t, 6), tC = __builtin_amdgcn_readlane(t, 7);
+        unsigned long long baseAR = 0ull, base12 = 0ull;
+        if (lane_id() == 0) {
+            const unsigned long long t1 = RT_QUEUE_ORDER ? tC : tL, t2 = RT_QUEUE_ORDER ? tL : tC;
+            unsigned long long* const pairs = (unsigned long long*)sa.outCounts;
+            if (tA | tR) baseAR = atomicAdd(pairs, (unsigned long long)tA | ((unsigned long long)tR << 32));
+            if (t1 | t2) base12 = atomicAdd(pairs + 1, t1 | (t2 << 32));
+            ShadeStatStripe* const st = sa.stats + (blockIdx.x & (RT_STAT_STRIPES - 1u));
+            atomicAdd(&st->raysReference, (unsigned long long)tRef);
+            if (tP) atomicAdd(&st->paths, (unsigned long long)tP);
+            atomicAdd(&st->segments, (unsigned long long)tS);
+            if (tE) atomicAdd(&st->emitterTests, (unsigned long long)tE);
+        }
+        const uint32_t bA = __builtin_amdgcn_readlane((uint32_t)baseAR, 0), bR = __builtin_amdgcn_readlane((uint32_t)(baseAR >> 32), 0);
+        const uint32_t b1 = __builtin_amdgcn_readlane((uint32_t)base12, 0), b2 = __builtin_amdgcn_readlane((uint32_t)(base12 >> 32), 0);
+        const uint32_t bL = RT_QUEUE_ORDER ? 2u * sa.auxOffset + b2 : sa.auxOffset + b1, bC = RT_QUEUE_ORDER ? sa.auxOffset + b1 : 2u * sa.auxOffset + b2;
+        if (lane_id() < 8u && (col < 2u || col > 5u)) {
+            uint32_t at = col == 0u ? bA : col == 1u ? bR : col == 6u ? bL : bC;
+            for (uint32_t r = 0; r < rows; r++) { const uint32_t v = s_cnt[r][col]; s_cnt[r][col] = at; at += v; }
+        }
     }
     __syncthreads();
-    if (alive) {
-        uint32_t baseA = s_base[0], baseR = s_base[1];
-        uint32_t baseX = (RT_QUEUE_ORDER ? 2u : 1u) * sa.auxOffset + s_base[2], baseY = (RT_QUEUE_ORDER ? 1u : 2u) * sa.auxOffset + s_base[3];
-        for (uint32_t w = 0; w < wv; w++) { baseA += s_cnt[w][0]; baseR += s_cnt[w][1]; baseX += s_cnt[w][6]; baseY += s_cnt[w][7]; }
-        sa.outActive[baseA + lanes_below(mAlive)] = slot;
-        if (!(auxMask & 4u)) sa.outRays[baseR + lanes_below(mM)] = (slot << 2) | ((auxMask & 8u) ? RAY_MAIN_BLANK : (uint32_t)RAY_MAIN);
-        if (auxMask & 1u) sa.outRays[baseX + lanes_below(mL)] = (slot << 2) | RAY_NEE;
-        if (auxMask & 2u) sa.outRays[baseY + lanes_below(mC)] = (slot << 2) | RAY_PROBE;
-    }
-}
-
-__global__ __launch_bounds__(RT_BLOCK) void k_shade(DevScene sc, PathState ps, ShadeArgs sa, FrameParams fp) { shade_block<false>(sc, ps, sa, fp); }
-__global__ __launch_bounds__(RT_BLOCK) void k_shade_maps(DevScene sc, PathState ps, ShadeArgs sa, FrameParams fp) { shade_block<true>(sc, ps, sa, fp); }
+#pragma unroll 1
+    for (uint32_t i = 0; i < iters; i++) {
+        const uint32_t k = kept >> (5u * i);
+        const bool alive = (k & 16u) != 0u;
+        const unsigned long long mAlive = __ballot(alive), mM = __ballot(alive && !(k & 4u));
+        const unsigned long long mL = __ballot(alive && (k & 1u)), mC = __ballot(alive && (k & 2u));
+        if (alive) {
+            const uint32_t* const row = s_cnt[i * (RT_BLOCK / RT_WAVE) + wv];
+            const uint32_t slot = sa.inActive[first + i * RT_BLOCK + threadIdx.x];
+            sa.outActive[row[0] + lanes_below(mAlive)] = slot;
+            if (!(k & 4u)) sa.outRays[row[1] + lanes_below(mM)] = (slot << 2) | ((k & 8u) ? RAY_MAIN_BLANK : (uint32_t)RAY_MAIN);
+            if (k & 1u) sa.outRays[row[6] + lanes_below(mL)] = (slot << 2) | RAY_NEE;
+            if (k & 2u) sa.outRays[row[7] + lanes_below(mC)] = (slot << 2) | RAY_PROBE;
+        }
+    }
+}
+
+__global__ __launch_bounds__(RT_BLOCK, 4) void k_shade(DevScene sc, PathState ps, ShadeArgs sa, FrameParams fp) { shade_block<false>(sc, ps, sa, fp); }
+__global__ __launch_bounds__(RT_BLOCK, 4) void k_shade_maps(DevScene sc, PathState ps, ShadeArgs sa, FrameParams fp) { shade_block<true>(sc, ps, sa, fp); }
 
 __device__ __forceinline__ rt_vec3 blend_frame(const FrameParams& fp, uint32_t frameCount, float4 oldc, float4 accum) {
     rt_vec3 out = f4xyz(accum);
@@ -1665,21 +1703,33 @@
 }
 
 __global__ void k_init_counts(uint32_t* counts, uint32_t n) {
-    if (threadIdx.x == 0) { counts[0] = n; counts[1] = 0; counts[2] = n; counts[3] = 0; counts[4] = 0; counts[5] = 0; counts[6] = 0; counts[7] = 0; counts[8] = 0; }
-}
-__global__ __launch_bounds__(RT_STAT_STRIPES) void k_fold_shade_stats(ShadeStatStripe* stats, DevCounters* counters) {
-    ShadeStatStripe* const st = stats + threadIdx.x;
-    const unsigned long long a = wave_sum_u64(st->raysReference), b = wave_sum_u64(st->paths), c = wave_sum_u64(st->segments), d = wave_sum_u64(st->emitterTests);
-    st->raysReference = 0; st->paths = 0; st->segments = 0; st->emitterTests = 0;
+    if (threadIdx.x < RT_CNT_WORDS) counts[threadIdx.x] = (threadIdx.x == RT_CNT_ACTIVE(0u) || threadIdx.x == RT_CNT_MAIN(0u)) ? n : 0u;
+}
+__global__ __launch_bounds__(RT_STAT_STRIPES) void k_fold_shade_stats(ShadeStatStripe* stats, TraceStatStripe* traceStats, DevCounters* counters) {
+    if (stats) {
+        ShadeStatStripe* const st = stats + threadIdx.x;
+        const unsigned long long a = wave_sum_u64(st->raysReference), b = wave_sum_u64(st->paths), c = wave_sum_u64(st->segments), d = wave_sum_u64(st->emitterTests);
+        st->raysReference = 0; st->paths = 0; st->segments = 0; st->emitterTests = 0;
+        if (lane_id() == 0) {
+            atomicAdd(&counters->raysReference, a);
+            atomicAdd(&counters->paths, b);
+            atomicAdd(&counters->segments, c);
+            atomicAdd(&counters->emitterTests, d);
+        }
+    }
+    TraceStatStripe* const ts = traceStats + threadIdx.x;
+    const unsigned long long a = wave_sum_u64(ts->boxTests), b = wave_sum_u64(ts->triTests), c = wave_sum_u64(ts->raysTraced), d = wave_sum_u64(ts->raysHit), e = wave_sum_u64(ts->skippedBoxTests);
+    ts->boxTests = 0; ts->triTests = 0; ts->raysTraced = 0; ts->raysHit = 0; ts->skippedBoxTests = 0;
     if (lane_id() == 0) {
-        atomicAdd(&counters->raysReference, a);
-        atomicAdd(&counters->paths, b);
-        atomicAdd(&counters->segments, c);
-        atomicAdd(&counters->emitterTests, d);
-    }
-}
-__global__ void k_zero_counts(uint32_t* a, uint32_t* b, uint32_t* c, uint32_t* d, uint32_t* e) {
-    if (threadIdx.x == 0) { *a = 0; *b = 0; *c = 0; *d = 0; *e = 0; }
+        atomicAdd(&counters->boxTests, a);
+        atomicAdd(&counters->triTests, b);
+        atomicAdd(&counters->raysTraced, c);
+        atomicAdd(&counters->raysHit, d);
+        if (e) atomicAdd(&counters->skippedBoxTests, e);
+    }
+}
+__global__ void k_zero_counts(uint32_t* counts, uint32_t p) {
+    if (threadIdx.x == 0) { counts[RT_CNT_ACTIVE(p)] = 0; counts[RT_CNT_MAIN(p)] = 0; counts[RT_CNT_AUX(p)] = 0; counts[RT_CNT_AUX2(p)] = 0; counts[RT_CNT_WORK] = 0; }
 }
 
 __device__ __host__ inline uint32_t selftest_mix(uint32_t h, float v) {
```

Measured after the change: 4757 Mrays/s (median of 6 runs). 7.5% higher.
